# yixuan/LBFGSpp

Measured on AMD Instinct MI355X. Metric: L-BFGS iterations/sec at n=10^8, m=10; achieved HBM GB/s vs peak, higher is better.
Workload: dtype f64; 1 GPU; north-star: extended Rosenbrock n=100000000 m=10 f64 LineSearchMoreThuente, x0 from counter hash; n=100000000, m=10, history_full=True, fevals_total=111, apply_Hv_persistent_launches=82

## Files before the change

include/LBFGSB.h:

```cpp
#ifndef LBFGSX_DROPIN_LBFGSB_H
#define LBFGSX_DROPIN_LBFGSB_H

#include <algorithm>
#include <cmath>
#include <limits>
#include <stdexcept>
#include <vector>

#include "LBFGSpp/BFGSMat.h"
#include "LBFGSpp/Cauchy.h"
#include "LBFGSpp/Device.h"
#include "LBFGSpp/Interop.h"
#include "LBFGSpp/LineSearchMoreThuente.h"
#include "LBFGSpp/Param.h"
#include "LBFGSpp/SubspaceMin.h"

namespace LBFGSpp {

template <typename Scalar, template <class> class LineSearch = LineSearchMoreThuente>
class LBFGSBSolver
{
    const LBFGSBParam<Scalar>& m_param;
    DeviceState<Scalar> m_dev;
    BFGSMatB<Scalar> m_bfgs;
// ... 69 lines not shown
        m_stats.gcp_total_s += gcp.t_total;
        detail::check(lbfgsx_b_dir_from_xcp(c, 1));
        constexpr Scalar eps = std::numeric_limits<Scalar>::epsilon();

        int k = 1;
        for (;;)
        {
            detail::Range range_iteration("lbfgsb:iteration");
            detail::check(lbfgsx_ls_begin(c));
            double dgd = 0, smax = 0;
            if (ev.builtin_id() >= 0 && !ev.reduce)
                detail::check(lbfgsx_b_dg_maxstep_trial(c, ev.builtin_id(), double(std::min(Scalar(1), m_param.max_step)), &dgd, &smax));
            else
                detail::check(lbfgsx_b_dg_maxstep(c, &dgd, &smax));
            Scalar dg = Scalar(dgd), step_max = Scalar(smax);
            if (dg >= Scalar(0) || step_max <= m_param.min_step)
            {
                detail::check(lbfgsx_b_dir_from_xcp(c, 0));
                m_bfgs.reset(c, m_param.m);
                detail::check(lbfgsx_b_dg_maxstep(c, &dgd, &smax));
                dg = Scalar(dgd);
                step_max = Scalar(smax);
                m_stats.resets++;
            }
            step_max = std::min(m_param.max_step, step_max);
            Scalar step = Scalar(1);
            step = std::min(step, step_max);
            const auto t_ls = std::chrono::steady_clock::now();
            ev.trial_written = false;
            try
            {
                detail::Range range_ls("lbfgsb:line_search");
                detail::run_line_search<Scalar, LineSearch<Scalar>, HostVec>(ev, m_param, step_max, step, fx, dg);
            }
            catch (...)
            {
                m_nfev = ev.nfev();
                if (ev.trial_written)
                    m_x_at_throw = LBFGSX_VEC_XT;
                throw;
            }
            m_nfev = ev.nfev();
            m_stats.linesearch_s += std::chrono::duration<double>(std::chrono::steady_clock::now() - t_ls).count();

            double pg = 0, x2 = 0, syd = 0, yyd = 0;
            detail::check(lbfgsx_b_post_linesearch_build(c, Cauchy<Scalar>::build_tau(gcp), &pg, &x2, &syd, &yyd));
            m_projgnorm = Scalar(pg);
            if (m_projgnorm <= m_param.epsilon || m_projgnorm <= m_param.epsilon_rel * sqrt(Scalar(x2)))
                return k;
            if (fpast > 0)
            {
                const Scalar old = m_fx[size_t(k % fpast)];
                if (k >= fpast && abs(old - fx) <= m_param.delta * std::max(std::max(abs(fx), abs(old)), Scalar(1)))
                    return k;
                m_fx[size_t(k % fpast)] = fx;
            }
            if (m_param.max_iterations != 0 && k >= m_param.max_iterations)
                return k;

            const auto t_corr = std::chrono::steady_clock::now();
            if (Scalar(syd) > eps * Scalar(yyd))
                m_bfgs.add_correction_begin(Scalar(syd), Scalar(yyd), m_defer_dots);
            m_stats.correction_s += std::chrono::duration<double>(std::chrono::steady_clock::now() - t_corr).count();

            detail::check(lbfgsx_b_force_bounds_deferred(c));
            {
                detail::Range range_gcp("lbfgsb:cauchy_point");
                Cauchy<Scalar>::get_cauchy_point(m_bfgs, gcp);
            }
            m_stats.gcp_crossings += gcp.crossings;
            m_stats.gcp_dev_crossings += gcp.dev_crossings;
            m_stats.gcp_sort_fallbacks = gcp.sort_fallbacks;
            m_stats.gcp_partial_sorts += (gcp.sorted < gcp.nord_total) ? 1 : 0;
            m_stats.gcp_searches++;
            m_stats.gcp_nord += gcp.nord_total;
            m_stats.gcp_sorted += gcp.sorted;
            m_stats.gcp_build_s += gcp.t_build;
            m_stats.gcp_fetch_s += gcp.t_fetch;
            m_stats.gcp_total_s += gcp.t_total;
            typename SubspaceMin<Scalar>::Stats st;
            const auto t_sub = std::chrono::steady_clock::now();
            {
                detail::Range range_sub("lbfgsb:subspace_min");
                SubspaceMin<Scalar>::subspace_minimize(m_bfgs, gcp, m_param.max_submin, &st);
            }
            m_stats.submin_s += std::chrono::duration<double>(std::chrono::steady_clock::now() - t_sub).count();
            m_stats.submin_calls++;
            m_stats.submin_sweeps += st.sweeps;
            m_stats.submin_unconverged += st.converged ? 0 : 1;
            m_stats.submin_fused_sweeps += st.fused_sweeps;
            m_stats.gram_carried = m_bfgs.carried_grams() - m_carried0;
            m_stats.rhs_identities = m_bfgs.rhs_identities() - m_ident0;
            if (m_trace_phases)
                std::fprintf(stderr, "[lbfgsb] it %d: ls %.3f ms (cum) corr %.3f gcp %.3f (build %.3f fetch %.3f) submin %.3f | crossings %lld dev %lld sweeps %lld\n",
                             k, m_stats.linesearch_s * 1e3, m_stats.correction_s * 1e3, m_stats.gcp_total_s * 1e3,
                             m_stats.gcp_build_s * 1e3, m_stats.gcp_fetch_s * 1e3, m_stats.submin_s * 1e3,
                             m_stats.gcp_crossings, m_stats.gcp_dev_crossings, m_stats.submin_sweeps);
            if (m_iter_hook)
                m_iter_hook(k);
            k++;
        }
    }
    const bool m_defer_dots = [] {
        const char* e = std::getenv("LBFGSX_CORR_DEFER");
        return !(e && e[0] == '0');
    }();
    const bool m_trace_phases = std::getenv("LBFGSX_TRACE_PHASES") != nullptr;

public:
    LBFGSBSolver(const LBFGSBParam<Scalar>& param) : m_param(param) { m_param.check_param(); }

    void set_device(int device) { m_device = device; }
    void set_trace(std::function<void(int, Scalar, DeviceState<Scalar>&)> cb) { m_trace = std::move(cb); }
    void set_iteration_hook(std::function<void(int)> cb) { m_iter_hook = std::move(cb); }
    DeviceState<Scalar>& device_state() { return m_dev; }
    int num_evaluations() const { return m_nfev; }
    const Stats& stats() const { return m_stats; }

    template <typename Foo, typename Vec>
    inline int minimize(Foo& f, Vec& x, Scalar& fx, const Vec& lb, const Vec& ub)
    {
        const std::int64_t n = std::int64_t(x.size());
        if (std::int64_t(lb.size()) != n || std::int64_t(ub.size()) != n)
            throw std::invalid_argument("'lb' and 'ub' must have the same size as 'x'");
        m_dev.ensure(n, m_param.m, LBFGSX_FLAG_BOUNDED, m_device);
        m_dev.upload(LBFGSX_VEC_X, x.data());
        m_dev.upload(LBFGSX_VEC_LB, lb.data());
        m_dev.upload(LBFGSX_VEC_UB, ub.data());
        int k = 0;
        m_x_at_throw = LBFGSX_VEC_X;
        try
        {
            k = run<Foo, Vec>(f, fx);
        }
        catch (...)
        {
            (void) lbfgsx_download(m_dev.ctx(), m_x_at_throw, x.data());
            throw;
        }
        m_dev.download(LBFGSX_VEC_X, x.data());
        return k;
    }

    template <typename Foo>
    inline int minimize_resident(Foo& f, std::int64_t n, Scalar& fx)
    {
        m_dev.ensure(n, m_param.m, LBFGSX_FLAG_BOUNDED, m_device);
        return run<Foo, std::vector<Scalar> >(f, fx);
    }
    void prepare_resident(std::int64_t n)
    {
        m_dev.ensure(n, m_param.m, LBFGSX_FLAG_BOUNDED, m_device);
        detail::check(lbfgsx_b_reserve(m_dev.ctx()));
    }

    const detail::ResultVector<Scalar>& final_grad() const
    {
        m_grad_host.resize(m_dev.size());
        m_dev.download(LBFGSX_VEC_G, m_grad_host.data());
        return m_grad_host;
    }
    Scalar final_grad_norm() const { return m_projgnorm; }
};

}

#endif
```

include/LBFGSpp/SubspaceMin.h:

```cpp
#ifndef LBFGSX_DROPIN_SUBSPACE_MIN_H
#define LBFGSX_DROPIN_SUBSPACE_MIN_H

#include <cstdint>
#include <cstdlib>
#include <limits>
#include <vector>

#include "BFGSMat.h"
#include "Cauchy.h"

namespace LBFGSpp {

template <typename Scalar>
class SubspaceMin
{
    static bool linear_coef(const BFGSMatB<Scalar>& bfgs, const typename Cauchy<Scalar>::Result& gcp, std::vector<double>& coef)
    {
        const int nc = bfgs.num_corrections();
        if (nc < 1 || gcp.nact < 1 || gcp.nfree < 1)
            return false;
        std::vector<Scalar> rhs;
        if (gcp.nact <= gcp.nfree)
            bfgs.Wtv(LBFGSX_VS_DRT, LBFGSX_ST_NEWACT, false, rhs);
        else
        {
            bfgs.Wtv(LBFGSX_VS_DRT, LBFGSX_ST_FREE, false, rhs);
            for (int j = 0; j < 2 * nc; j++)
                rhs[size_t(j)] = gcp.vecc[size_t(j)] - rhs[size_t(j)];
        }
        bfgs.Mv_scaled(rhs, coef);
        return true;
    }

    static bool PtBQv_coef(const BFGSMatB<Scalar>& bfgs, int qmask, int vsel, std::int64_t nP, std::int64_t nQ,
                           std::vector<double>& coef)
    {
        if (bfgs.num_corrections() < 1 || nP < 1 || nQ < 1)
            return false;
        std::vector<Scalar> WQtv;
        std::int64_t nnz = 0;
        bfgs.Wtv(vsel, qmask, false, WQtv, &nnz);
        if (nnz < 1)
            return false;
        bfgs.Mv_scaled(WQtv, coef);
        return true;
    }

public:
    struct Stats
    {
        int sweeps = 0;
        bool converged = true;
        int fused_sweeps = 0;
    };

    static void subspace_minimize(const BFGSMatB<Scalar>& bfgs, const typename Cauchy<Scalar>::Result& gcp, int maxit,
                                  Stats* stats = nullptr)
    {
        lbfgsx_ctx* c = bfgs.ctx();
        const Scalar theta = bfgs.theta();
        detail::check(lbfgsx_b_sub_begin(c));
        const std::int64_t nfree = gcp.nfree;
        if (nfree < 1)
            return;

        std::vector<double> lcoef;
        const bool has_lin = linear_coef(bfgs, gcp, lcoef);
        bfgs.gram_cache_reset();
        const char* fuse_env = std::getenv("LBFGSX_SUB_FUSE");
        const bool fuse = !(fuse_env && fuse_env[0] == '0');
        const char* os_env = std::getenv("LBFGSX_LU_ONE_SIDED");
        const bool one_sided = !(os_env && os_env[0] == '0');
        std::int64_t s7[7] = {0, 0, 0, 0, 0, 0, 0};
        bool swept = false;
        if (fuse)
            detail::check(lbfgsx_b_set_compaction(c, 1));
        bfgs.solve_PtBP(LBFGSX_ST_FREE, nfree, LBFGSX_VS_NEG_CF, LBFGSX_GP_LINEAR,
                        has_lin ? lcoef.data() : nullptr, nullptr, nullptr, 0,
                        true, 0, -1, fuse ? s7 : nullptr, true, &swept);
        std::int64_t cnt[4];
        std::int64_t nL = 0, nU = 0, nP = 0;
        auto take = [&](const std::int64_t* a, const std::int64_t* b2) {
            nL = a[0] + (b2 ? b2[0] : 0);
            nU = a[1] + (b2 ? b2[1] : 0);
            nP = a[2] + (b2 ? b2[2] : 0);
            for (int q = 0; q < 4; q++)
                cnt[q] = a[3 + q] + (b2 ? b2[3 + q] : 0);
        };
        int nfused = swept ? 1 : 0;
        if (swept)
            take(s7, nullptr);
        else if (fuse)
            detail::check(lbfgsx_b_sub_sweep_begin(c, 1, &nL, &nU, &nP, cnt));
        else
            detail::check(lbfgsx_b_sub_check(c, cnt));
        if (cnt[0] == 0)
        {
            detail::check(lbfgsx_b_sub_op(c, LBFGSX_SO_ASSIGN_Y));
            return;
        }
        if (!fuse)
            detail::check(lbfgsx_b_sub_op(c, LBFGSX_SO_SAVE_FALLBACK));

        int k;
        for (k = 0; k < maxit; k++)
        {
            swept = false;
            if (!fuse)
            {
                detail::check(lbfgsx_b_sub_partition(c, &nL, &nU, &nP));
                if (nP > 0)
                    detail::check(lbfgsx_b_sub_op(c, LBFGSX_SO_RHS_INIT));
            }
            const bool need_mult = (nL > 0 || nU > 0);
            std::vector<Scalar> Fy;
            bool have_Fy = false;
            if (nP > 0)
            {
                std::vector<double> cl, cu;
                bool hasL, hasU;
                std::vector<Scalar> wl, wu;
                std::int64_t zl = 0, zu = 0;
                if ((one_sided ? (nL > 0 || nU > 0) : (nL > 0 && nU > 0)) && bfgs.Wtv_lu(wl, zl, wu, zu))
                {
                    hasL = zl >= 1;
                    hasU = zu >= 1;
                    if (hasL)
                        bfgs.Mv_scaled(wl, cl);
                    if (hasU)
                        bfgs.Mv_scaled(wu, cu);
                }
                else
                {
                    hasL = PtBQv_coef(bfgs, LBFGSX_ST_L, LBFGSX_VS_LBOUND, nP, nL, cl);
                    hasU = PtBQv_coef(bfgs, LBFGSX_ST_U, LBFGSX_VS_UBOUND, nP, nU, cu);
                }
                bfgs.solve_PtBP(LBFGSX_ST_P, nP, LBFGSX_VS_NEG_RHS, (hasL || hasU) ? LBFGSX_GP_RHS : LBFGSX_GP_NONE,
                                hasL ? cl.data() : nullptr, hasU ? cu.data() : nullptr, need_mult ? &Fy : nullptr,
                                LBFGSX_ST_FREE, false, LBFGSX_ST_L | LBFGSX_ST_U, nL + nU,
                                (fuse && need_mult && k + 1 < maxit) ? s7 : nullptr, false, &swept);
                have_Fy = need_mult;
            }
            if (need_mult)
            {
                if (!have_Fy)
                    bfgs.Wtv(LBFGSX_VS_Y, LBFGSX_ST_FREE, false, Fy);
                std::vector<double> coef;
                bfgs.Mv_scaled(Fy, coef);
                const double* cf = (bfgs.num_corrections() < 1) ? nullptr : coef.data();
                if (swept)
                {
                    std::int64_t t7[7];
                    detail::check(lbfgsx_b_lu_sweep(c, cf, double(theta), t7));
                    take(s7, t7);
                    nfused++;
// ... 50 lines not shown
```

include/lbfgsx.h:

```cpp
#ifndef LBFGSX_H
#define LBFGSX_H

#include <stddef.h>
#include <stdint.h>

#ifdef __cplusplus
extern "C" {
#endif

typedef struct lbfgsx_ctx lbfgsx_ctx;

enum { LBFGSX_F64 = 0, LBFGSX_F32 = 1 };
enum { LBFGSX_OBJ_NONE = -1, LBFGSX_OBJ_DIAG_QUAD = 0, LBFGSX_OBJ_EXT_ROSENBROCK = 1,
       LBFGSX_OBJ_BOUND = 64  };
enum
{
    LBFGSX_OK = 0,
    LBFGSX_E_INVALID = -1,
    LBFGSX_E_LOGIC = -2,
    LBFGSX_E_RUNTIME = -3,
    LBFGSX_E_HIP = -4,
    LBFGSX_E_NOGPU = -5,
    LBFGSX_E_USER = -6
};
// ... 42 lines not shown
int lbfgsx_bfgs_download_history(lbfgsx_ctx* c, void* S_out, void* Y_out, int* ncorr, int* ptr, double* theta);
int lbfgsx_apply_Hv(lbfgsx_ctx* c, int v_which, double a, double* dg);

int lbfgsx_eval(lbfgsx_ctx* c, int objective, double* fx, double* gnorm2, double* xnorm2);
int lbfgsx_norms(lbfgsx_ctx* c, double* gnorm2, double* xnorm2);
int lbfgsx_ls_begin(lbfgsx_ctx* c);
int lbfgsx_trial(lbfgsx_ctx* c, int objective, double step, double* fx, double* dg);
int lbfgsx_trial_point(lbfgsx_ctx* c, double step);
int lbfgsx_trial_dg(lbfgsx_ctx* c, double* dg);
int lbfgsx_ls_keep_trial_as_lo(lbfgsx_ctx* c);
int lbfgsx_ls_end(lbfgsx_ctx* c, int use_lo);
int lbfgsx_post_linesearch(lbfgsx_ctx* c, double* gnorm2, double* xnorm2, double* sy, double* yy);
int lbfgsx_commit_correction(lbfgsx_ctx* c);
int lbfgsx_post_linesearch_spec(lbfgsx_ctx* c, double a, double* gnorm2, double* xnorm2, double* sy, double* yy);
int lbfgsx_spec_counts(const lbfgsx_ctx* c, int64_t out[3]);
typedef struct lbfgsx_objective lbfgsx_objective;
int lbfgsx_objective_compile(lbfgsx_objective** out, int dtype, int K, const char* body, char* log, size_t log_len);
void lbfgsx_objective_destroy(lbfgsx_objective* obj);
long long lbfgsx_objective_source(int dtype, int K, const char* body, char* out, size_t len);
int lbfgsx_objective_info(const lbfgsx_objective* obj, long long out[8]);
int lbfgsx_objective_K(const lbfgsx_objective* obj);
int lbfgsx_objective_dtype(const lbfgsx_objective* obj);
int lbfgsx_objective_bind(lbfgsx_ctx* c, const lbfgsx_objective* obj, const void* const p[4], const double cs[8], int* id);
int lbfgsx_objective_upload(lbfgsx_ctx* c, int slot, const void* host, void** dev);
int lbfgsx_objective_bound(const lbfgsx_ctx* c, const void* p[4]);
enum { LBFGSX_FORM_TERM = 0, LBFGSX_FORM_CHAIN = 1, LBFGSX_FORM_GRID = 2 };
int lbfgsx_objective_compile_chain(lbfgsx_objective** out, int dtype, int K, const char* body, char* log, size_t log_len);
long long lbfgsx_objective_source_chain(int dtype, int K, const char* body, char* out, size_t len);
int lbfgsx_objective_form(const lbfgsx_objective* obj);
int lbfgsx_objective_compile_grid(lbfgsx_objective** out, int dtype, const char* body, char* log, size_t log_len);
long long lbfgsx_objective_source_grid(int dtype, const char* body, char* out, size_t len);
int lbfgsx_objective_bind_grid(lbfgsx_ctx* c, const lbfgsx_objective* obj, int64_t rows, int64_t cols, const void* const p[4],
                               const double cs[8], int* id);
int lbfgsx_objective_shape(const lbfgsx_ctx* c, int64_t* rows, int64_t* cols);
int lbfgsx_device(const lbfgsx_ctx* c);
int lbfgsx_device_push(const lbfgsx_ctx* c, int* prev);
int lbfgsx_device_pop(int prev);
int lbfgsx_persist_counts(const lbfgsx_ctx* c, int64_t out[4]);
int lbfgsx_debug_persist_fault(lbfgsx_ctx* c);
int lbfgsx_counters(int64_t out[3], int reset);
int lbfgsx_counters_ex(int64_t out[8], int reset);
int lbfgsx_poll_counts(const lbfgsx_ctx* c, int64_t out[2]);
int lbfgsx_poll_counts_ex(const lbfgsx_ctx* c, int64_t out[4]);
void lbfgsx_range_push(const char* name);
void lbfgsx_range_pop(void);

int lbfgsx_gs_post_linesearch(lbfgsx_ctx* c, double scal[7], double* sdots, double* gdots, double* ydots);
int lbfgsx_gs_set_history_dtype(lbfgsx_ctx* c, int dtype);
int lbfgsx_gs_direction(lbfgsx_ctx* c, const double* coef, double coef_g, double* dg);

enum
{
    LBFGSX_ST_FREE = 1, LBFGSX_ST_NEWACT = 2, LBFGSX_ST_L = 4, LBFGSX_ST_U = 8, LBFGSX_ST_P = 16
};
enum
{
    LBFGSX_VS_DRT = 0,
    LBFGSX_VS_NEG_CF = 1,
    LBFGSX_VS_NEG_RHS = 2,
    LBFGSX_VS_LBOUND = 3,
    LBFGSX_VS_UBOUND = 4,
    LBFGSX_VS_Y = 5
};
enum
{
    LBFGSX_CB_LINEAR = 0,
    LBFGSX_CB_SOLVE = 1,
    LBFGSX_CB_RHS_ADD = 2,
    LBFGSX_CB_LAMBDA = 3,
    LBFGSX_CB_MU = 4
};
enum
{
    LBFGSX_SO_SAVE_FALLBACK = 0, LBFGSX_SO_RHS_INIT = 1, LBFGSX_SO_ASSIGN_Y = 2, LBFGSX_SO_CLAMP_Y = 3,
    LBFGSX_SO_CLAMP_FB = 4, LBFGSX_SO_ASSIGN_FB = 5
};
int lbfgsx_b_force_bounds(lbfgsx_ctx* c);
int lbfgsx_b_force_bounds_deferred(lbfgsx_ctx* c);
int lbfgsx_b_eval(lbfgsx_ctx* c, int objective, double* fx, double* projgnorm, double* xnorm2);
int lbfgsx_b_norms(lbfgsx_ctx* c, double* projgnorm, double* xnorm2);
int lbfgsx_b_dg_maxstep(lbfgsx_ctx* c, double* dg, double* step_max);
int lbfgsx_b_dg_maxstep_trial(lbfgsx_ctx* c, int objective, double step0, double* dg, double* step_max);
int lbfgsx_b_trial_ahead_counts(const lbfgsx_ctx* c, int64_t out[2]);
int lbfgsx_b_post_linesearch(lbfgsx_ctx* c, double* projgnorm, double* xnorm2, double* sy, double* yy);
int lbfgsx_b_post_linesearch_build(lbfgsx_ctx* c, double tau, double* projgnorm, double* xnorm2, double* sy, double* yy);
int lbfgsx_b_post_build_counts(int64_t out[2], int reset);
int lbfgsx_b_psel_counts(int64_t out[1], int reset);
int lbfgsx_b_correction_dots(lbfgsx_ctx* c, double* sdots, double* ydots);
int lbfgsx_b_correction_dots_defer(lbfgsx_ctx* c);
int lbfgsx_b_cauchy_build(lbfgsx_ctx* c, int64_t* nfree, int64_t* nord, double* dd, double* wtd);
int lbfgsx_b_cauchy_chunk(lbfgsx_ctx* c, int64_t first, int64_t count, double* brk, double* g, double* z, int* idx,
                          double* wrows);
int lbfgsx_b_cauchy_build_partial(lbfgsx_ctx* c, double tau, int64_t* nfree, int64_t* nord, int64_t* nsorted, double* dd,
                                  double* wtd);
int lbfgsx_b_cauchy_sort_full(lbfgsx_ctx* c);
int lbfgsx_b_cauchy_scan(lbfgsx_ctx* ctx, int64_t first, int64_t count, int64_t nord, const double* Mmat, double theta,
                         double t_prev, const double* state_in, int64_t* exit_at, double* state_out);
int lbfgsx_b_cauchy_finish(lbfgsx_ctx* c, double t_cross, double tfinal, int crossed_all, int64_t* nact, int64_t* nfree);
int lbfgsx_b_sub_begin(lbfgsx_ctx* c);
int lbfgsx_b_wtv(lbfgsx_ctx* c, int vsel, int mask, double* out, int64_t* nnz);
int lbfgsx_b_gram(lbfgsx_ctx* c, int mask, double* gram);
int lbfgsx_b_gram_fused(lbfgsx_ctx* c, int mask, int vsel, double* gram, double* wtv);
enum { LBFGSX_GP_NONE = 0, LBFGSX_GP_RHS = 1, LBFGSX_GP_LINEAR = 2 };
int lbfgsx_b_gram_fused_ex(lbfgsx_ctx* c, int mask, int vsel_id, int prologue, const double* coef1, const double* coef2,
                           double* gram, double* wtv);
int lbfgsx_b_gram_fused_dd(lbfgsx_ctx* c, int mask, int vsel_id, int prologue, const double* coef1, const double* coef2,
                           double* gram, double* wtv, double* gram_dd);
int lbfgsx_b_wtv_prologue(lbfgsx_ctx* c, int mask, int vsel_id, int prologue, const double* coef1, const double* coef2,
                          double* wtv);
int lbfgsx_b_solve_wty(lbfgsx_ctx* c, int pmask, int vsel, const double* coef, double theta, int fmask, double* wty);
int lbfgsx_b_wcombine(lbfgsx_ctx* c, int mode, int mask, int vsel, const double* coef, double theta);
int lbfgsx_b_sub_partition(lbfgsx_ctx* c, int64_t* nL, int64_t* nU, int64_t* nP);
int lbfgsx_b_sub_check(lbfgsx_ctx* c, int64_t counts[4]);
int lbfgsx_b_sub_sweep_begin(lbfgsx_ctx* c, int first, int64_t* nL, int64_t* nU, int64_t* nP, int64_t counts[4]);
int lbfgsx_b_wtv_lu(lbfgsx_ctx* c, double* out_l, int64_t* nnz_l, double* out_u, int64_t* nnz_u);
int lbfgsx_b_wtv_lu_c(lbfgsx_ctx* c, double* out_l, int64_t* nnz_l, double* out_u, int64_t* nnz_u, double* negc_dd);
int lbfgsx_b_free_delta(lbfgsx_ctx* c, int64_t* n_enter, int64_t* n_leave);
int lbfgsx_b_gram_list_dd(lbfgsx_ctx* c, int which, double* gram_dd);
int lbfgsx_b_gram_pairs_dd(lbfgsx_ctx* c, int mask, int vsel, int prologue, const double* coef1, const double* coef2,
                           int npairs, const int* pair_i, const int* pair_j, int refresh_slot, double* out_dd);
int lbfgsx_b_gram_pairs_max(lbfgsx_ctx* c);
int lbfgsx_b_gram_last_vrow_dd(lbfgsx_ctx* c, double* out_dd);
int lbfgsx_b_set_compaction(lbfgsx_ctx* c, int enable);
int lbfgsx_b_compact_vec_counts(int64_t out[4], int reset);
int lbfgsx_b_reserve(lbfgsx_ctx* c);
int lbfgsx_b_solve_sweep(lbfgsx_ctx* c, int first, int vsel, const double* coef, double theta, double* wty, int64_t sums[7]);
int lbfgsx_b_solve_sweep_rhs(lbfgsx_ctx* c, int first, int vsel, const double* coef, double theta, const double* rhs_c1,
                             const double* rhs_c2, double* wty, int64_t sums[7]);
int lbfgsx_b_solve_sweep_rhs_ready(lbfgsx_ctx* c);
int lbfgsx_b_lu_sweep(lbfgsx_ctx* c, const double* coef, double theta, int64_t sums[7]);
int lbfgsx_b_sub_op(lbfgsx_ctx* c, int op);
int lbfgsx_b_download_state(lbfgsx_ctx* c, unsigned char* host);
int lbfgsx_b_dot_drt_g(lbfgsx_ctx* c, double* dg);
int lbfgsx_b_dir_from_xcp(lbfgsx_ctx* c, int normalize);

typedef struct lbfgsx_batch lbfgsx_batch;
typedef struct
{
    int active;
    int mode;
    int x_in;
    int x_out;
    int col_u;
    int col_w;
    int i_num, i_den, i_num2, i_theta, i_out;
    float pad;
    double step;
} lbfgsx_bat_desc;
enum
{
    LBFGSX_BAT_EVAL = 0, LBFGSX_BAT_TRIAL = 1, LBFGSX_BAT_POST = 2, LBFGSX_BAT_TWOLOOP = 3,
    LBFGSX_BAT_POINT = 4, LBFGSX_BAT_GDOT = 5, LBFGSX_BAT_NORMS = 6
};
typedef struct
{
    int active;
    int x_in;
    int ncorr;
    int pcol[32];
} lbfgsx_bat_hvdesc;
enum
{
    LBFGSX_BAT_IT_POST = 1,
    LBFGSX_BAT_IT_POST_ONLY = 2,
    LBFGSX_BAT_IT_TRIAL = 4,
    LBFGSX_BAT_IT_TRIAL_ONLY = 8
// ... 73 lines not shown
```

lbfgspp_amd/_lib.py:

```python
import ctypes as C
import os

HERE = os.path.dirname(os.path.abspath(__file__))

F64, F32 = 0, 1
OBJ_DIAG_QUAD, OBJ_EXT_ROSENBROCK = 0, 1
OBJ_BOUND = 64
LS_NOCEDAL_WRIGHT, LS_MORE_THUENTE, LS_BACKTRACKING, LS_BRACKETING = 0, 1, 2, 3
ALGO_LBFGS, ALGO_LBFGSB = 0, 1
RECURSION_VECTOR, RECURSION_GRAM_SPACE, RECURSION_GRAM_SPACE_F32H = 0, 1, 2
FLAG_BOUNDED = 1
(VEC_X, VEC_G, VEC_XP, VEC_GP, VEC_D, VEC_XT, VEC_GT, VEC_A, VEC_B, VEC_LB, VEC_UB, VEC_XCP) = range(12)
E_INVALID, E_LOGIC, E_RUNTIME, E_HIP, E_NOGPU, E_USER = -1, -2, -3, -4, -5, -6


class Params(C.Structure):
    _fields_ = [("m", C.c_int), ("epsilon", C.c_double), ("epsilon_rel", C.c_double), ("past", C.c_int),
                ("delta", C.c_double), ("max_iterations", C.c_int), ("linesearch", C.c_int),
                ("max_linesearch", C.c_int), ("min_step", C.c_double), ("max_step", C.c_double),
                ("ftol", C.c_double), ("wolfe", C.c_double), ("max_submin", C.c_int)]


class Result(C.Structure):
    _fields_ = [("niter", C.c_int), ("nfev", C.c_int), ("fx", C.c_double), ("gnorm", C.c_double),
# ... 46 lines not shown
        f = getattr(lib, name)
        f.restype = res
        f.argtypes = list(args)
        return f

    sig(core, "lbfgsx_last_error", C.c_char_p)
    sig(core, "lbfgsx_version", C.c_char_p)
    sig(core, "lbfgsx_device_count", i32)
    sig(core, "lbfgsx_create", i32, C.POINTER(vp), i32, i64, i32, i32, i32)
    sig(core, "lbfgsx_destroy", None, vp)
    sig(core, "lbfgsx_set_stream", i32, vp, vp)
    sig(core, "lbfgsx_sync", i32, vp)
    sig(core, "lbfgsx_n", i64, vp)
    sig(core, "lbfgsx_vec", vp, vp, i32)
    sig(core, "lbfgsx_upload", i32, vp, i32, vp)
    sig(core, "lbfgsx_download", i32, vp, i32, vp)
    sig(core, "lbfgsx_gather", i32, vp, i32, i64, pd)
    sig(core, "lbfgsx_gen_diag_quad", i32, vp, dbl, C.c_uint64)
    sig(core, "lbfgsx_gen_rosen_x0", i32, vp, C.c_uint64)
    sig(core, "lbfgsx_fill", i32, vp, i32, dbl)
    sig(core, "lbfgsx_bfgs_reset", i32, vp)
    sig(core, "lbfgsx_bfgs_ncorr", i32, vp)
    sig(core, "lbfgsx_bfgs_theta", dbl, vp)
    sig(core, "lbfgsx_bfgs_add_correction_host", i32, vp, vp, vp)
    sig(core, "lbfgsx_bfgs_download_history", i32, vp, vp, vp, C.POINTER(i32), C.POINTER(i32), pd)
    sig(core, "lbfgsx_apply_Hv", i32, vp, i32, dbl, pd)
    sig(core, "lbfgsx_eval", i32, vp, i32, pd, pd, pd)
    sig(core, "lbfgsx_norms", i32, vp, pd, pd)
    sig(core, "lbfgsx_ls_begin", i32, vp)
    sig(core, "lbfgsx_trial", i32, vp, i32, dbl, pd, pd)
    sig(core, "lbfgsx_trial_point", i32, vp, dbl)
    sig(core, "lbfgsx_trial_dg", i32, vp, pd)
    sig(core, "lbfgsx_ls_keep_trial_as_lo", i32, vp)
    sig(core, "lbfgsx_ls_end", i32, vp, i32)
    sig(core, "lbfgsx_post_linesearch", i32, vp, pd, pd, pd, pd)
    sig(core, "lbfgsx_commit_correction", i32, vp)
    sig(core, "lbfgsx_gs_post_linesearch", i32, vp, pd, pd, pd, pd)
    sig(core, "lbfgsx_gs_set_history_dtype", i32, vp, i32)
    sig(core, "lbfgsx_gs_direction", i32, vp, pd, dbl, pd)
    sig(core, "lbfgsx_timing_enable", i32, vp, i32)
    sig(core, "lbfgsx_timing_read", i32, vp, pd, C.POINTER(i64), pd, C.POINTER(i64))
    sig(core, "lbfgsx_stream_probe", i32, vp, i32, pd, pd)
    sig(core, "lbfgsx_selftest_reduce", i32, vp, i32, i32, i32, pd)
    sig(core, "lbfgsx_post_linesearch_spec", i32, vp, dbl, pd, pd, pd, pd)
    sig(core, "lbfgsx_rccl_allgather_records", i32, C.POINTER(i32), i32, vp, i64, i64, C.POINTER(vp))
    sig(core, "lbfgsx_device_download", i32, i32, vp, i64, vp)
    sig(core, "lbfgsx_device_free", None, i32, vp)
    sig(core, "lbfgsx_spec_counts", i32, vp, C.POINTER(i64 * 3))
    sig(core, "lbfgsx_counters", i32, C.POINTER(i64 * 3), i32)
    sig(core, "lbfgsx_counters_ex", i32, C.POINTER(i64 * 8), i32)
    sig(core, "lbfgsx_poll_counts", i32, vp, C.POINTER(i64 * 2))
    sig(core, "lbfgsx_poll_counts_ex", i32, vp, C.POINTER(i64 * 4))
    sig(core, "lbfgsx_b_compact_vec_counts", i32, C.POINTER(i64 * 4), i32)
    sig(core, "lbfgsx_b_reserve", i32, vp)
    sig(core, "lbfgsx_device", i32, vp)
    sig(core, "lbfgsx_persist_counts", i32, vp, C.POINTER(i64 * 4))
    sig(core, "lbfgsx_debug_persist_fault", i32, vp)

    sig(sol, "lbfgsx_solver_create", i32, C.POINTER(vp), i32, i32, i32, C.POINTER(Params), i32)
    sig(sol, "lbfgsx_solver_create_error", C.c_char_p)
    sig(sol, "lbfgsx_solver_destroy", None, vp)
    sig(sol, "lbfgsx_solver_prepare", i32, vp, i64)
    sig(sol, "lbfgsx_solver_ctx", vp, vp)
    sig(sol, "lbfgsx_solver_set_recursion", i32, vp, i32)
    sig(sol, "lbfgsx_solver_set_allreduce", i32, vp, ALLREDUCE, vp)
    sig(sol, "lbfgsx_solver_set_devices", i32, vp, C.POINTER(i32), i32)
    sig(core, "lbfgsx_comm_unique_id", i32, C.c_char_p)
    sig(core, "lbfgsx_comm_create_rank", i32, C.POINTER(vp), i32, i32, i32, C.c_char_p)
    sig(core, "lbfgsx_comm_create_local", i32, C.POINTER(vp), C.POINTER(i32), i32)
    sig(core, "lbfgsx_comm_allreduce_sum", i32, vp, i32, pd, i32)
    sig(core, "lbfgsx_comm_abort", i32, vp)
    sig(core, "lbfgsx_comm_abort_from", i32, vp, i32)
    sig(core, "lbfgsx_comm_first_abort", i32, vp)
    sig(core, "lbfgsx_b_gram_pairs_max", i32, vp)
    sig(core, "lbfgsx_b_post_linesearch_build", i32, vp, dbl, pd, pd, pd, pd)
    sig(core, "lbfgsx_b_post_build_counts", i32, C.POINTER(i64 * 2), i32)
    sig(core, "lbfgsx_b_psel_counts", i32, C.POINTER(i64 * 1), i32)
    sig(core, "lbfgsx_b_dg_maxstep_trial", i32, vp, i32, dbl, pd, pd)
    sig(core, "lbfgsx_b_solve_sweep_rhs", i32, vp, i32, i32, pd, dbl, pd, pd, pd, C.POINTER(i64 * 7))
    sig(core, "lbfgsx_b_solve_sweep_rhs_ready", i32, vp)
    sig(core, "lbfgsx_b_gram_last_vrow_dd", i32, vp, pd)
    sig(core, "lbfgsx_b_wtv_lu_c", i32, vp, pd, C.POINTER(i64), pd, C.POINTER(i64), pd)
    sig(core, "lbfgsx_b_trial_ahead_counts", i32, vp, C.POINTER(i64 * 2))
    sig(core, "lbfgsx_comm_info", i32, vp, C.POINTER(i32 * 4))
    sig(core, "lbfgsx_comm_calls", i64, vp, i32)
    sig(core, "lbfgsx_comm_hook_arg", vp, vp, i32)
    sig(core, "lbfgsx_comm_destroy", None, vp)
    sig(core, "lbfgsx_set_shard", i32, vp, i64, i64)
    sig(sol, "lbfgsx_solver_set_iteration_hook", i32, vp, ITER_HOOK, vp)
    sig(sol, "lbfgsx_batch_minimize", i32, i32, i32, i32, C.POINTER(Params), i32, i64, i64, i64, C.c_uint64, i32, i32,
        C.POINTER(BatchItem))
    sig(sol, "lbfgsx_batch_minimize_lockstep", i32, i32, C.POINTER(Params), i64, i64, i32, C.c_uint64, i32,
        C.POINTER(BatchItem), vp, C.c_char_p, i32)
    sig(sol, "lbfgsx_batch_minimize_lockstep_multi", i32, i32, C.POINTER(Params), i64, i64, i32, C.c_uint64,
        C.POINTER(i32), i32, C.POINTER(BatchItem), vp, C.c_char_p, i32)
    sig(sol, "lbfgsx_batch_minimize_lockstep_ex", i32, i32, i32, i32, dbl, C.POINTER(Params), i64, i64, i32, C.c_uint64,
        C.POINTER(i32), i32, C.POINTER(BatchItem), vp, C.c_char_p, i32)
    sig(sol, "lbfgsx_lockstep_create", i32, C.POINTER(vp), i32, i32, C.POINTER(Params), i64, i32, i32, i32, C.c_char_p, i32)
    sig(sol, "lbfgsx_lockstep_minimize", i32, vp, i32, dbl, C.c_uint64, i64, C.POINTER(BatchItem), vp, C.POINTER(dbl * 8),
        C.c_char_p, i32)
    sig(sol, "lbfgsx_lockstep_destroy", None, vp)
    sig(sol, "lbfgsx_lockstep_set_timing", i32, vp, i32)
    sig(sol, "lbfgsx_solver_hessians", i32, vp, vp, vp)
    sig(sol, "lbfgsx_solver_stats", i32, vp, C.POINTER(C.c_longlong * 8))
    sig(sol, "lbfgsx_solver_stats2", i32, vp, C.POINTER(C.c_longlong * 8))
    sig(sol, "lbfgsx_solver_stats3", i32, vp, C.POINTER(C.c_longlong * 8))
    sig(sol, "lbfgsx_solver_minimize", i32, vp, i32, i64, vp, vp, vp, vp, vp, C.POINTER(Trace), C.POINTER(Result))
    sig(sol, "lbfgsx_solver_minimize_fn", i32, vp, i64, OBJECTIVE_FN, vp, vp, vp, vp, C.POINTER(Trace), C.POINTER(Result))
    sig(sol, "lbfgsx_lockstep_minimize_fn", i32, vp, vp, BATCH_OBJECTIVE_FN, vp, C.POINTER(BatchItem), vp, C.POINTER(dbl * 8),
        C.c_char_p, i32)
    sig(core, "lbfgsx_objective_compile", i32, C.POINTER(vp), i32, i32, C.c_char_p, C.c_char_p, C.c_size_t)
    sig(core, "lbfgsx_objective_destroy", None, vp)
    sig(core, "lbfgsx_objective_source", C.c_longlong, i32, i32, C.c_char_p, C.c_char_p, C.c_size_t)
    sig(core, "lbfgsx_objective_info", i32, vp, C.POINTER(C.c_longlong * 8))
    sig(core, "lbfgsx_objective_compile_chain", i32, C.POINTER(vp), i32, i32, C.c_char_p, C.c_char_p, C.c_size_t)
    sig(core, "lbfgsx_objective_source_chain", C.c_longlong, i32, i32, C.c_char_p, C.c_char_p, C.c_size_t)
    sig(core, "lbfgsx_objective_form", i32, vp)
    sig(core, "lbfgsx_objective_K", i32, vp)
    sig(core, "lbfgsx_objective_dtype", i32, vp)
    sig(core, "lbfgsx_objective_bind", i32, vp, vp, C.POINTER(vp * 4), C.POINTER(dbl * 8), C.POINTER(i32))
    sig(core, "lbfgsx_objective_upload", i32, vp, i32, vp, C.POINTER(vp))
    sig(core, "lbfgsx_objective_bound", i32, vp, C.POINTER(vp * 4))
    sig(sol, "lbfgsx_solver_minimize_obj", i32, vp, vp, i64, C.POINTER(vp * 4), i32, C.POINTER(dbl * 8), vp, vp, vp,
        C.POINTER(Trace), C.POINTER(Result))
    sig(core, "lbfgsx_objective_compile_grid", i32, C.POINTER(vp), i32, C.c_char_p, C.c_char_p, C.c_size_t)
    sig(core, "lbfgsx_objective_source_grid", C.c_longlong, i32, C.c_char_p, C.c_char_p, C.c_size_t)
    sig(core, "lbfgsx_objective_bind_grid", i32, vp, vp, i64, i64, C.POINTER(vp * 4), C.POINTER(dbl * 8), C.POINTER(i32))
    sig(core, "lbfgsx_objective_shape", i32, vp, C.POINTER(i64), C.POINTER(i64))
    sig(sol, "lbfgsx_solver_minimize_grid", i32, vp, vp, i64, i64, C.POINTER(vp * 4), i32, C.POINTER(dbl * 8), vp, vp, vp,
        C.POINTER(Trace), C.POINTER(Result))
    _core, _solver = core, sol
    return core, sol


def last_error():
    core, _ = load()
    return core.lbfgsx_last_error().decode()


_EXC = {E_INVALID: ValueError, E_LOGIC: ArithmeticError, E_RUNTIME: RuntimeError, E_HIP: RuntimeError,
        E_NOGPU: RuntimeError, E_USER: RuntimeError}


def check(rc, msg=None):
    if rc != 0:
        raise _EXC.get(rc, RuntimeError)(msg if msg is not None else last_error())


def require_torch(who):
    try:
        import torch
    except ImportError as e:
        raise ImportError("%s needs PyTorch (ROCm build): its callable receives torch tensors that alias the library's "
                          "device vectors" % who) from e
    return torch


class _DeviceMemory:

    def __init__(self, ptr, shape, np_dtype, strides):
        import numpy as np
        self.__cuda_array_interface__ = {"shape": tuple(shape), "typestr": np.dtype(np_dtype).str, "data": (int(ptr), False),
                                         "version": 2, "strides": strides}


def device_tensor(ptr, shape, np_dtype, device, row_stride=None):
# ... 6 lines not shown
```

lbfgspp_amd/csrc/lbfgsb.hip:

```cpp
#include <algorithm>
#include <atomic>
#include <cmath>
#include <cstdlib>
#include <cstdio>
#include <cstring>

#define LBFGSB_TU "lbfgsb"
#include "lbfgsb_state.hpp"

namespace lbfgsx {

static std::atomic<int64_t> g_cv_starts{0}, g_cv_backs{0}, g_wtdc_runs{0}, g_stash_hits{0};
void count_cv_start() { g_cv_starts.fetch_add(1, std::memory_order_relaxed); }
void count_wtdc_run() { g_wtdc_runs.fetch_add(1, std::memory_order_relaxed); }
void count_stash_hit() { g_stash_hits.fetch_add(1, std::memory_order_relaxed); }

int cv_alloc(lbfgsx_ctx* c)
{
    lbfgsb_state* b = c->bstate;
    if (b->cv_buf && b->cv_cap >= c->ld)
        return LBFGSX_OK;
    if (b->cv_buf)
        (void) hipFree(b->cv_buf);
    b->cv_buf = nullptr;
// ... 92 lines not shown
int fetch_T(lbfgsx_ctx* c, int idx, int k, double* out)
{
    if (idx == c->sl.out(0) && c->outmap_dev)
    {
        LBFGSX_HIP(lbfgsx::poll_wait(c));
        const volatile T* h = static_cast<const volatile T*>(c->outmap_host);
        for (int i = 0; i < k; i++)
            out[i] = double(h[i]);
        return LBFGSX_OK;
    }
    LBFGSX_HIP(lbfgsx::copy_async(c->hout, P<T>(c->sc) + idx, sizeof(T) * size_t(k), hipMemcpyDeviceToHost, c->stream));
    LBFGSX_HIP(lbfgsx::stream_sync(c->stream));
    const T* h = static_cast<const T*>(c->hout);
    for (int i = 0; i < k; i++)
        out[i] = double(h[i]);
    return LBFGSX_OK;
}

template int fetch_T<float>(lbfgsx_ctx*, int, int, double*);
template int fetch_T<double>(lbfgsx_ctx*, int, int, double*);

int bounded_alloc(lbfgsx_ctx* c)
{
    lbfgsb_state* b = new lbfgsb_state();
    c->bstate = b;
    const size_t vbytes = size_t(c->ld) * c->esz;
    void** vecs[] = {&b->brk, &b->dvec, &b->cF, &b->y, &b->yfb, &b->lam, &b->mu, &b->rhs, &b->keys_in, &b->keys_out};
    for (void** v : vecs)
        LBFGSX_HIP(hipMalloc(v, vbytes));
    LBFGSX_HIP(hipMalloc(reinterpret_cast<void**>(&b->st), size_t(c->ld)));
    LBFGSX_HIP(hipMemset(b->st, 0, size_t(c->ld)));
    LBFGSX_HIP(hipMalloc(reinterpret_cast<void**>(&b->vals_in), sizeof(int) * size_t(c->ld)));
    LBFGSX_HIP(hipMalloc(reinterpret_cast<void**>(&b->vals_out), sizeof(int) * size_t(c->ld)));
    LBFGSX_HIP(hipMalloc(reinterpret_cast<void**>(&b->phys_dev), sizeof(int) * size_t(c->m + 1)));
    if (c->outmap_dev)
    {
        LBFGSX_HIP(hipHostMalloc(reinterpret_cast<void**>(&b->dout_host), sizeof(double) * lbfgsb_state::kDout, hipHostMallocMapped | hipHostMallocCoherent));
        std::memset(b->dout_host, 0, sizeof(double) * lbfgsb_state::kDout);
        LBFGSX_HIP(hipHostGetDevicePointer(reinterpret_cast<void**>(&b->dout), b->dout_host, 0));
    }
    else
        LBFGSX_HIP(hipMalloc(reinterpret_cast<void**>(&b->dout), sizeof(double) * lbfgsb_state::kDout));
    LBFGSX_HIP(hipMalloc(&b->coef_dev, sizeof(double) * 80));
    b->lu_cap = unsigned(std::min<int64_t>(c->n, int64_t(1) << 20));
    LBFGSX_HIP(hipMalloc(reinterpret_cast<void**>(&b->lu_list), sizeof(int) * 2 * size_t(b->lu_cap)));
    LBFGSX_HIP(hipMalloc(reinterpret_cast<void**>(&b->lu_cnt), sizeof(unsigned)));
    LBFGSX_HIP(hipMemset(b->lu_cnt, 0, sizeof(unsigned)));
    if (const char* e = getenv("LBFGSX_SWEEP_SOLVE_FUSE"))
        b->sweep_fuse = atoi(e) != 0;
    if (const char* e = getenv("LBFGSX_COMPACT_FREE"))
        b->wf_use = atoi(e) != 0;
    if (const char* e = getenv("LBFGSX_SPLIT"))
        b->split = atoi(e) != 0;
    if (const char* e = getenv("LBFGSX_FINISH_FUSE"))
        b->fin_fuse = atoi(e) != 0;
    if (const char* e = getenv("LBFGSX_NEWACT_CAP"))
        b->na_cap = unsigned(std::max(1, std::min(1 << 20, atoi(e))));
    LBFGSX_HIP(hipMalloc(reinterpret_cast<void**>(&b->na_list), sizeof(int) * size_t(b->na_cap)));
    LBFGSX_HIP(hipMalloc(reinterpret_cast<void**>(&b->na_cnt), sizeof(unsigned)));
    LBFGSX_HIP(hipMemset(b->na_cnt, 0, sizeof(unsigned)));
    LBFGSX_HIP(hipMalloc(reinterpret_cast<void**>(&b->xp1), sizeof(double) * size_t(kMaxGridX) * kMaxSumsX * 2));
    LBFGSX_HIP(hipMalloc(reinterpret_cast<void**>(&b->xp2), sizeof(double) * size_t(kMaxGridX / kGroupX) * kMaxSumsX * 2));
    LBFGSX_HIP(hipMalloc(reinterpret_cast<void**>(&b->xtickets), sizeof(unsigned) * (2 + kMaxGridX / kGroupX)));
    LBFGSX_HIP(hipMemset(b->xtickets, 0, sizeof(unsigned) * (2 + kMaxGridX / kGroupX)));
    b->gtile = std::max(3, xl::gram_kpb(2 * c->m + 1));
    if (const char* e = getenv("LBFGSX_COMPACT_VEC"))
        b->cv_use = atoi(e) != 0;
    if (const char* e = getenv("LBFGSX_WTD_COMPACT"))
        b->wtdc_use = atoi(e) != 0;
    if (const char* e = getenv("LBFGSX_SELECT_INLINE"))
        b->psel_use = atoi(e) != 0;
    if (const char* e = getenv("LBFGSX_POST_BUILD"))
        b->pb_use = atoi(e) != 0;
    if (const char* e = getenv("LBFGSX_TRIAL_AHEAD"))
        b->st_use = atoi(e) != 0;
    if (const char* e = getenv("LBFGSX_RHS_IDENTITY"))
        b->rhs_identity = atoi(e) != 0;
    if (const char* e = getenv("LBFGSX_CHUNK_AHEAD"))
        b->gpre_use = atoi(e) != 0;
    if (const char* e = getenv("LBFGSX_DELTA_AHEAD"))
        b->fd_use = atoi(e) != 0;
    if (const char* e = getenv("LBFGSX_LIST12"))
        b->list12 = atoi(e) != 0;
    if (const char* e = getenv("LBFGSX_PSEL_SMALL"))
        b->psel_small = atoi(e) != 0;
    if (const char* e = getenv("LBFGSX_SELECT_CAP"))
        b->psel_cap = unsigned(std::max(1, std::min(1 << 24, atoi(e))));
    if (const char* e = getenv("LBFGSX_SYNC_MERGE"))
        b->stash_use = atoi(e) != 0;
    if (const char* e = getenv("LBFGSX_WTD_LIST_CAP"))
        b->wtdc_cap = unsigned(std::max(1, std::min(1 << 20, atoi(e))));
    LBFGSX_HIP(hipMalloc(reinterpret_cast<void**>(&b->colmax), sizeof(unsigned long long) * 2 * size_t(c->m + 1)));
    LBFGSX_HIP(hipMemset(b->colmax, 0, sizeof(unsigned long long) * 2 * size_t(c->m + 1)));
    b->colmax_ok.assign(size_t(c->m + 1), 0);
    const size_t bytes = sort_pairs_tmp_bytes(c);
    if (const char* e = getenv("LBFGSX_GRAM"))
    {
        b->gram_i8 = (std::strcmp(e, "i8") == 0);
        if (const char* e2 = getenv("LBFGSX_GRAM_I8_MIN"))
            b->i8_min_tot = std::max(1, atoi(e2));
        b->gram_mode = (std::strcmp(e, "blocked") == 0) ? 2 : 0;
        if (!b->gram_i8 && b->gram_mode == 0 && e[0] != 0 && std::strcmp(e, "dd") != 0)
        {
            static bool warned = false;
            if (!warned)
                fprintf(stderr, "lbfgsx: LBFGSX_GRAM=%s is not a Gram kernel (i8, blocked, dd): using the default\n", e);
            warned = true;
        }
    }
    if (const char* e = getenv("LBFGSX_GCP_CHAIN"))
        b->chain_host = std::strcmp(e, "scan") != 0;
    if (const char* e = getenv("LBFGSX_MULTIDOT"))
        b->multidot_chunked = (std::strcmp(e, "chunked") == 0);
    {
        hipDeviceProp_t prop;
        if (hipGetDeviceProperties(&prop, c->device) == hipSuccess && prop.multiProcessorCount > 0)
            b->num_cus = prop.multiProcessorCount;
    }
    const size_t gent = size_t(b->gtile) * 256;
    LBFGSX_HIP(hipMalloc(reinterpret_cast<void**>(&b->gram_partial), sizeof(double) * size_t(lbfgsb_state::kGramBlocks) * gent * 2));
    LBFGSX_HIP(hipMalloc(reinterpret_cast<void**>(&b->gram_partial2), sizeof(double) * 32 * gent * 2));
    if (c->outmap_dev)
    {
        LBFGSX_HIP(hipHostMalloc(reinterpret_cast<void**>(&b->gram_dd_host), sizeof(double) * gent * 2, hipHostMallocMapped | hipHostMallocCoherent));
        LBFGSX_HIP(hipHostGetDevicePointer(reinterpret_cast<void**>(&b->gram_dd), b->gram_dd_host, 0));
        LBFGSX_HIP(hipHostMalloc(reinterpret_cast<void**>(&b->stash_host), sizeof(double) * 3 * (gent * 3), hipHostMallocMapped | hipHostMallocCoherent));
        LBFGSX_HIP(hipHostGetDevicePointer(reinterpret_cast<void**>(&b->stash_dev), b->stash_host, 0));
        LBFGSX_HIP(hipHostMalloc(reinterpret_cast<void**>(&b->gram_out_host), sizeof(double) * gent, hipHostMallocMapped | hipHostMallocCoherent));
        LBFGSX_HIP(hipHostGetDevicePointer(reinterpret_cast<void**>(&b->gram_out), b->gram_out_host, 0));
    }
    else
    {
        LBFGSX_HIP(hipMalloc(reinterpret_cast<void**>(&b->gram_out), sizeof(double) * gent));
        LBFGSX_HIP(hipMalloc(reinterpret_cast<void**>(&b->gram_dd), sizeof(double) * gent * 2));
    }
    b->sort_tmp_bytes = bytes;
    LBFGSX_HIP(hipMalloc(&b->sort_tmp, bytes ? bytes : 16));
    return LBFGSX_OK;
}

void bounded_free(lbfgsx_ctx* c)
{
    lbfgsb_state* b = c->bstate;
    if (!b)
        return;
    void* ptrs[] = {b->brk, b->dvec, b->cF, b->y, b->yfb, b->lam, b->mu, b->rhs, b->keys_in, b->keys_out, b->st,
                    b->vals_in, b->vals_out, b->phys_dev, b->dout, b->coef_dev, b->sort_tmp, b->g_brk,
                    b->g_g, b->g_z, b->g_w, b->g_idx, b->gram_partial, b->gram_partial2, b->gram_out, b->gram_dd,
                    b->s_brk, b->s_g, b->s_z, b->s_W, b->s_P, b->s_C, b->s_chain, b->s_ts, b->s_off,
                    b->s_small, b->s_exit, b->pk, b->pv, b->pcount, b->sel_tmp};
    if (b->h_chain)
        (void) hipHostFree(b->h_chain);
    if (b->exit_map_host)
        (void) hipHostFree(b->exit_map_host);
    if (b->gout_host)
        (void) hipHostFree(b->gout_host);
    if (b->g_host)
        (void) hipHostFree(b->g_host);
    if (b->fd_host)
        (void) hipHostFree(b->fd_host);
    (void) hipFree(b->lu_list);
    (void) hipFree(b->wf_pos);
    (void) hipFree(b->wtdc_list);
    (void) hipFree(b->wtdc_cnt);
    (void) hipFree(b->psel_list);
    (void) hipFree(b->psel_cnt);
    (void) hipFree(b->psel_tmp);
    for (hipEvent_t ev : b->chain_ev)
        if (ev)
            (void) hipEventDestroy(ev);
    (void) hipFree(b->fprev);
    (void) hipFree(b->dl_enter);
    (void) hipFree(b->dl_leave);
    (void) hipFree(b->dl_cnt);
    (void) hipFree(b->wf);
    (void) hipFree(b->wf_idx);
    (void) hipFree(b->wf_cnt);
    (void) hipFree(b->wf_base);
    (void) hipFree(b->wf_tmp);
    (void) hipFree(b->lu_cnt);
    (void) hipFree(b->colmax);
    (void) hipFree(b->i8_part);
    (void) hipFree(b->i8_partv);
    (void) hipFree(b->i8_vsum);
    for (void* p : ptrs)
    {
        if ((p == b->dout && b->dout_host) || (p == b->gram_out && b->gram_out_host) || (p == b->gram_dd && b->gram_dd_host))
            continue;
        (void) hipFree(p);
    }
    if (b->dout_host)
        (void) hipHostFree(b->dout_host);
    if (b->gram_out_host)
        (void) hipHostFree(b->gram_out_host);
    if (b->gram_dd_host)
        (void) hipHostFree(b->gram_dd_host);
    if (b->stash_host)
        (void) hipHostFree(b->stash_host);
    (void) hipFree(b->cv_buf);
    (void) hipFree(b->na_list);
    (void) hipFree(b->na_cnt);
    (void) hipFree(b->xp1);
    (void) hipFree(b->xp2);
    (void) hipFree(b->xtickets);
    delete b;
    c->bstate = nullptr;
}

RedWsX wsx(lbfgsx_ctx* c)
{
    RedWsX w;
    w.p1 = c->bstate->xp1;
    w.p2 = c->bstate->xp2;
    w.tickets = c->bstate->xtickets;
    w.done = c->ws.done;
    w.seq = c->ws.seq;
    return w;
}
int ensure_keys(lbfgsx_ctx* c)
{
    lbfgsb_state* b = c->bstate;
    if (b->keys_valid && b->vals_iota)
        return LBFGSX_OK;
    const int grid = c->grid_for(c->n);
    DISPATCH_T(c, {
        lbfgsx::model_add(double(c->n) * (2 * sizeof(T) + (b->vals_iota ? 0 : 4)));
        LBFGSX_LAUNCH((k_keys_from_brk<T>), dim3(grid), dim3(kBlock), 0, c->stream, static_cast<const T*>(b->brk),
                      static_cast<T*>(b->keys_in), b->vals_iota ? static_cast<int*>(nullptr) : b->vals_in, c->n);
    });
    LBFGSX_HIP(hipGetLastError());
    b->keys_valid = true;
    b->vals_iota = true;
    return LBFGSX_OK;
}

void wf_rebuilt(lbfgsx_ctx* c)
{
    lbfgsb_state* b = c->bstate;
    b->wf_valid = true;
    b->wf_n = b->nfree_last;
    b->wf_live = true;
    b->wf_ncorr = c->ncorr;
    b->wf_epoch = b->sub_epoch;
}

bool wtdc_ready(lbfgsx_ctx* c, bool assume_defer)
{
    lbfgsb_state* b = c->bstate;
    const int total = 2 * c->ncorr;
    return b->wtdc_use && (b->corr_defer || assume_defer) && (b->split ? (total >= 2 && total <= kColsX) : (total > 8 && total <= 20)) &&
           !b->multidot_chunked && b->wf_use && b->wf_live &&
           (b->wf_ncorr == c->ncorr || b->wf_ncorr + 1 == c->ncorr) && b->wf_epoch == b->sub_epoch && c->n < (int64_t(1) << 31) &&
           b->wf_n >= 4096 && b->wf_n * 4 <= c->n * 3;
}
bool wtdc_prepare(lbfgsx_ctx* c)
{
    lbfgsb_state* b = c->bstate;
    b->wtdc_n = -1;
    if (!wtdc_ready(c))
        return false;
    return wtdc_alloc(c);
}
bool wtdc_alloc(lbfgsx_ctx* c)
{
    lbfgsb_state* b = c->bstate;
    if (!b->wtdc_list)
    {
        if (hipMalloc(reinterpret_cast<void**>(&b->wtdc_list), sizeof(int) * size_t(b->wtdc_cap)) != hipSuccess ||
            hipMalloc(reinterpret_cast<void**>(&b->wtdc_cnt), sizeof(unsigned)) != hipSuccess ||
            hipMemsetAsync(b->wtdc_cnt, 0, sizeof(unsigned), c->stream) != hipSuccess)
        {
            (void) hipGetLastError();
            (void) hipFree(b->wtdc_list);
            (void) hipFree(b->wtdc_cnt);
            b->wtdc_list = nullptr;
            b->wtdc_cnt = nullptr;
            b->wtdc_use = false;
            return false;
        }
    }
    return true;
}

int run_force_bounds(lbfgsx_ctx* c)
{
    c->bstate->pb_valid = false;
    lbfgsx::DeviceGuard dev_guard_(c->device);
    const int grid = c->grid_for(c->n);
    DISPATCH_T(c, {
        LBFGSX_LAUNCH((k_force_bounds<T>), dim3(grid), dim3(kBlock), 0, c->stream, P<T>(c->xb[c->cur]), P<T>(c->lb),
                           P<T>(c->ub), c->n);
    });
    LBFGSX_HIP(hipGetLastError());
    return LBFGSX_OK;
}

int psort_alloc(lbfgsx_ctx* c)
{
    lbfgsb_state* b = c->bstate;
    if (!b->pk)
    {
        const size_t n = size_t(c->n);
        LBFGSX_HIP(hipMalloc(&b->pk, c->esz * n));
        LBFGSX_HIP(hipMalloc(reinterpret_cast<void**>(&b->pv), sizeof(int) * n));
        LBFGSX_HIP(hipMalloc(reinterpret_cast<void**>(&b->pcount), sizeof(unsigned)));
    }
    return LBFGSX_OK;
}

int delta_alloc(lbfgsx_ctx* c)
{
    lbfgsb_state* b = c->bstate;
    if (!b->fprev)
    {
        b->dl_cap = unsigned(std::min<int64_t>(c->n, std::max<int64_t>(int64_t(1) << 14, std::min<int64_t>(int64_t(1) << 20, c->n / 64))));
        LBFGSX_HIP(hipMalloc(reinterpret_cast<void**>(&b->fprev), size_t(c->ld)));
        LBFGSX_HIP(hipMemsetAsync(b->fprev, 0, size_t(c->ld), c->stream));
        LBFGSX_HIP(hipMalloc(reinterpret_cast<void**>(&b->dl_enter), sizeof(int) * size_t(b->dl_cap)));
        LBFGSX_HIP(hipMalloc(reinterpret_cast<void**>(&b->dl_leave), sizeof(int) * size_t(b->dl_cap)));
        LBFGSX_HIP(hipMalloc(reinterpret_cast<void**>(&b->dl_cnt), sizeof(unsigned) * 4));
    }
    return LBFGSX_OK;
}

}

using namespace lbfgsx;

extern "C" {

int lbfgsx_b_reserve(lbfgsx_ctx* c)
{
    lbfgsx::DeviceGuard dev_guard_(c->device);
    int rc = need_bounded(c);
    if (rc)
        return rc;
    lbfgsb_state* b = c->bstate;
    const int m2 = 2 * c->m;
    const int ncap = m2 <= 32 ? std::max(4, (m2 + 3) / 4 * 4) : m2 <= 40 ? 40 : m2 <= 48 ? 48 : m2 <= 64 ? 64 : 80;
    if (m2 <= 80)
    {
        rc = scan_alloc(c, std::min<int64_t>(int64_t(1) << 20, c->n), ncap);
        if (rc)
            return rc;
    }
    rc = psort_alloc(c);
    if (rc)
        return rc;
    rc = delta_alloc(c);
    if (rc)
        return rc;
    if (b->wf_use && c->n >= 4096 && c->n < (int64_t(1) << 31))
        (void) wf_alloc(c);
    if (b->cv_use && b->wf_use)
        (void) cv_alloc(c);
    if (b->wtdc_use)
        (void) wtdc_alloc(c);
    return LBFGSX_OK;
}

int lbfgsx_b_compact_vec_counts(int64_t out[4], int reset)
{
    if (out)
    {
        out[0] = g_cv_starts.load(std::memory_order_relaxed);
        out[1] = g_cv_backs.load(std::memory_order_relaxed);
        out[2] = g_wtdc_runs.load(std::memory_order_relaxed);
        out[3] = g_stash_hits.load(std::memory_order_relaxed);
    }
    if (reset)
    {
        g_cv_starts = 0;
        g_cv_backs = 0;
        g_wtdc_runs = 0;
        g_stash_hits = 0;
    }
    return LBFGSX_OK;
}

int lbfgsx_b_set_compaction(lbfgsx_ctx* c, int enable)
{
    int rc = need_bounded(c);
    if (rc)
        return rc;
    c->bstate->wf_on = enable != 0;
    if (!enable)
        c->bstate->wf_valid = false;
    return LBFGSX_OK;
}

int lbfgsx_b_download_state(lbfgsx_ctx* c, unsigned char* host)
{
    lbfgsx::DeviceGuard dev_guard_(c->device);
    int rc = need_bounded(c);
    if (rc)
        return rc;
    LBFGSX_HIP(lbfgsx::copy_async(host, c->bstate->st, size_t(c->n), hipMemcpyDeviceToHost, c->stream));
    LBFGSX_HIP(lbfgsx::stream_sync(c->stream));
    return LBFGSX_OK;
}

}
```

lbfgspp_amd/csrc/lbfgsb_cauchy.hip:

```cpp
#include <algorithm>
#include <atomic>
#include <cmath>
#include <cstdlib>
#include <cstdio>
#include <cstring>

#include <rocprim/rocprim.hpp>

#include "gcp_scan.cuh"

#define LBFGSB_TU "lbfgsb_cauchy"
#include "lbfgsb_state.hpp"

namespace lbfgsx {

template <class T>
struct KeyLE
{
    T tau;
    __device__ bool operator()(const T& k) const { return k <= tau; }
};
template <class T>
__global__ void k_gather_keys(const T* __restrict__ keys, const int* __restrict__ idx, T* __restrict__ out, int64_t count)
{
// ... 202 lines not shown
        b->psel_list = nullptr;
        b->psel_cnt = nullptr;
        b->psel_tmp = nullptr;
        b->psel_use = false;
        return false;
    }
    b->psel_tmp_bytes = bytes;
    return true;
}
template <class T>
static int partial_sort_tail_t(lbfgsx_ctx* c, unsigned cnt, int64_t* nsorted)
{
    lbfgsb_state* b = c->bstate;
    *nsorted = int64_t(cnt);
    if (cnt == 0)
        return LBFGSX_OK;
    const int grid = int(std::min<int64_t>((int64_t(cnt) + 255) / 256, 1024));
    LBFGSX_LAUNCH((k_gather_keys<T>), dim3(grid), dim3(256), 0, c->stream, b->keys_valid ? P<T>(b->keys_in) : static_cast<T*>(b->brk),
                  b->pv, P<T>(b->pk), int64_t(cnt));
    size_t sbytes = b->sort_tmp_bytes;
    lbfgsx::model_add(double(cnt) * (96.0 + 64.0 + 2 * sizeof(T)));
    LBFGSX_HIP(rocprim::radix_sort_pairs(b->sort_tmp, sbytes, P<T>(b->pk), P<T>(b->keys_out), b->pv, b->vals_out, size_t(cnt), 0,
                                         int(sizeof(T) * 8), c->stream));
    return LBFGSX_OK;
}
template <class T>
static int partial_sort_listed_t(lbfgsx_ctx* c, unsigned cnt, int64_t* nsorted)
{
    lbfgsb_state* b = c->bstate;
    if (b->psel_small && cnt >= 1 && cnt <= unsigned(kPselSmallCap))
    {
        *nsorted = int64_t(cnt);
        g_psel_small++;
        lbfgsx::model_add(double(cnt) * (64.0 + 4 + 2 * (sizeof(T) + 4)));
        LBFGSX_LAUNCH((k_psel_sort_small<T>), dim3(1), dim3(kPselSmallThreads), 0, c->stream, b->psel_list, int(cnt),
                      b->keys_valid ? P<T>(b->keys_in) : static_cast<T*>(b->brk), P<T>(b->keys_out), b->vals_out);
        LBFGSX_HIP(hipGetLastError());
        return LBFGSX_OK;
    }
    if (cnt > 1)
    {
        size_t bytes = b->psel_tmp_bytes;
        int end_bit = 1;
        while (end_bit < 32 && (int64_t(1) << end_bit) < c->n)
            end_bit++;
        LBFGSX_HIP(rocprim::radix_sort_keys(b->psel_tmp, bytes, b->psel_list, b->pv, size_t(cnt), 0, end_bit, c->stream));
    }
    else if (cnt == 1)
        LBFGSX_HIP(lbfgsx::copy_async(b->pv, b->psel_list, sizeof(int), hipMemcpyDeviceToDevice, c->stream));
    return partial_sort_tail_t<T>(c, cnt, nsorted);
}
template <class T>
static int partial_sort_t(lbfgsx_ctx* c, double tau, int64_t* nsorted)
{
    lbfgsb_state* b = c->bstate;
    int rc = partial_select_t<T>(c, tau, nullptr);
    if (rc)
        return rc;
    unsigned cnt = 0;
    LBFGSX_HIP(lbfgsx::copy_async(&cnt, b->pcount, sizeof(unsigned), hipMemcpyDeviceToHost, c->stream));
    LBFGSX_HIP(lbfgsx::stream_sync(c->stream));
    return partial_sort_tail_t<T>(c, cnt, nsorted);
}
static int cauchy_chunk_launch(lbfgsx_ctx* c, int64_t first, int64_t count, bool with_w, int* idx, double** land,
                               std::vector<double>* pageable)
{
    lbfgsb_state* b = c->bstate;
    const int nc = c->ncorr;
    const size_t per = size_t(3 + 2 * nc);
    const size_t per_cap = size_t(3 + 2 * c->m);
    if (count > b->g_cap || c->m != b->g_ncorr)
    {
        void* old[] = {b->g_brk, b->g_idx};
        for (void* p : old)
            (void) hipFree(p);
        b->g_brk = nullptr;
        b->g_idx = nullptr;
        const int64_t cap = std::max<int64_t>(count, b->g_cap);
        LBFGSX_HIP(hipMalloc(reinterpret_cast<void**>(&b->g_brk), sizeof(double) * size_t(cap) * per_cap));
        LBFGSX_HIP(hipMalloc(reinterpret_cast<void**>(&b->g_idx), sizeof(int) * size_t(cap)));
        b->g_cap = cap;
        b->g_ncorr = c->m;
    }
    double* d_brk = b->g_brk;
    double* d_g = d_brk + count;
    double* d_z = d_g + count;
    double* d_w = d_z + count;
    int rc = upload_phys(c);
    if (rc)
        return rc;
    const int grid = int(std::min<int64_t>((count + 255) / 256, 2048));
    DISPATCH_T(c, {
        BVecs<T> bv = bvecs<T>(c);
        LBFGSX_LAUNCH((k_cauchy_gather<T>), dim3(grid), dim3(256), 0, c->stream, bv, P<T>(b->keys_out), b->vals_out, first,
                           count, P<T>(c->S), P<T>(c->Y), c->ld, b->phys_dev, nc, d_brk, d_g, d_z, b->g_idx, d_w);
    });
    LBFGSX_HIP(hipGetLastError());
    const size_t ndbl = size_t(count) * ((nc > 0 && with_w) ? per : size_t(3));
    if (ndbl > b->g_host_cap)
    {
        if (b->g_host)
            (void) hipHostFree(b->g_host);
        b->g_host = nullptr;
        b->g_host_cap = 0;
        const size_t want = std::max<size_t>(ndbl, size_t(1) << 16);
        if (want <= (size_t(1) << 25))
        {
            LBFGSX_HIP(hipHostMalloc(reinterpret_cast<void**>(&b->g_host), sizeof(double) * want, hipHostMallocDefault));
            b->g_host_cap = want;
        }
    }
    *land = b->g_host;
    if (ndbl > b->g_host_cap)
    {
        if (!pageable)
            return LBFGSX_E_INVALID;
        pageable->resize(ndbl);
        *land = pageable->data();
    }
    LBFGSX_HIP(lbfgsx::copy_async(*land, d_brk, sizeof(double) * ndbl, hipMemcpyDeviceToHost, c->stream));
    if (idx)
        LBFGSX_HIP(lbfgsx::copy_async(idx, b->g_idx, sizeof(int) * size_t(count), hipMemcpyDeviceToHost, c->stream));
    return LBFGSX_OK;
}
template <int NC>
static int gcp_scan_nc(lbfgsx_ctx* c, const GcpBufs& gb, int64_t first, int64_t count, int64_t nord, double theta,
                       double t_prev)
{
    lbfgsb_state* b = c->bstate;
    const int nc = c->ncorr;
    const int ntiles = int((count + kGcpTile - 1) / kGcpTile);
    double* M = b->s_small;
    double* initA = M + NC * NC;
    double* initB = initA + NC;
    double* initC = initB + NC + 1;
    double* fin = initC + 1;
    double* out = fin + NC + 1;
    hipStream_t st = c->stream;
    LBFGSX_LAUNCH((k_gcp_a1<NC>), dim3(ntiles), dim3(kGcpTile), 0, st, gb, count, nc, theta, b->s_ts);
    LBFGSX_LAUNCH(k_gcp_tiles, dim3(NC), dim3(64), 0, st, b->s_ts, b->s_off, ntiles, NC, initA, fin);
    LBFGSX_LAUNCH((k_gcp_a3b1<NC>), dim3(ntiles), dim3(kGcpTile), 0, st, gb, count, nc, theta, t_prev, M, b->s_off, b->s_ts);
    LBFGSX_LAUNCH(k_gcp_tiles, dim3(NC + 1), dim3(64), 0, st, b->s_ts, b->s_off, ntiles, NC + 1, initB, fin);
    if (b->chain_host)
    {
        LBFGSX_LAUNCH((k_gcp_b3c1<NC, true>), dim3(ntiles), dim3(kGcpTile), 0, st, gb, count, nc, theta, t_prev, M,
                           b->s_off, b->s_ts, first, nord);
        LBFGSX_HIP(hipGetLastError());
        return LBFGSX_OK;
    }
    LBFGSX_LAUNCH((k_gcp_b3c1<NC, false>), dim3(ntiles), dim3(kGcpTile), 0, st, gb, count, nc, theta, t_prev, M, b->s_off, b->s_ts, first, nord);
    LBFGSX_LAUNCH(k_gcp_tiles, dim3(1), dim3(64), 0, st, b->s_ts, b->s_off, ntiles, 1, initC, fin);
    LBFGSX_LAUNCH(k_gcp_c3, dim3(ntiles), dim3(kGcpTile), 0, st, gb, count, first, nord, b->s_off, b->s_exit);
    LBFGSX_LAUNCH((k_gcp_extract<NC>), dim3(1), dim3(64), 0, st, gb, count, nc, theta, b->s_exit, out);
    LBFGSX_HIP(hipGetLastError());
    return LBFGSX_OK;
}
template <int NC>
static void gcp_extract_nc(lbfgsx_ctx* c, const GcpBufs& gb, int64_t count, double theta)
{
    lbfgsb_state* b = c->bstate;
    LBFGSX_LAUNCH((k_gcp_extract<NC>), dim3(1), dim3(64), 0, c->stream, gb, count, c->ncorr, theta, b->exit_map_dev, b->gout_dev);
}

template <class CT>
static int64_t gcp_chain_host(const double* dt, const double* A, const double* B, int64_t k0, int64_t k1, double& fp, double& fpp)
{
    CT f1 = CT(fp), f2 = CT(fpp);
    for (int64_t k = k0; k < k1; k++)
    {
        f1 = f1 + CT(dt[k]) * f2;
        f1 = f1 + CT(A[k]);
        f2 = f2 - CT(B[k]);
        const CT dn = CT(dt[k + 1]);
        if (dn > CT(0) && !(-f1 / f2 >= dn))
        {
            fp = double(f1);
            fpp = double(f2);
            return k;
        }
    }
    fp = double(f1);
// ... 115 lines not shown
        return rc;
    lbfgsb_state* b = c->bstate;
    const bool force = b->force_pending;
    b->force_pending = false;
    const int grid = c->grid_for(c->n);
    double r[5] = {0, 0, 0, -1, -1};
    int64_t ns = 0;
    const bool tau_ok = tau > 0.0 && std::isfinite(tau);
    const bool sel_inline = tau_ok && b->psel_use && b->psel_last >= 0 && b->psel_last <= lbfgsb_state::kPselMax &&
                            c->n < (int64_t(1) << 31) && psel_alloc(c);
    const bool sel_ahead = !sel_inline && b->stash_use && b->dout_host && tau_ok;
    DISPATCH_T(c, {
        BVecs<T> bv = bvecs<T>(c);
        const bool wc = wtdc_prepare(c);
        const int newest = (c->ptr + c->m - 1) % c->m;
        const bool from_post = b->pb_valid && b->pb_cur == c->cur && b->pb_tau == tau && b->pb_sel_inline == sel_inline &&
                               b->pb_wc == wc && !sel_ahead && (!force || b->pb_r[5] == 0.0);
        b->pb_valid = false;
        if (from_post)
        {
            for (int i = 0; i < 5; i++)
                r[i] = b->pb_r[i];
            count_pb_hit();
        }
        else
        {
        if (!sel_ahead)
            lbfgsx::poll_arm(c);
        lbfgsx::model_add(double(c->n) * (7 * sizeof(T) + 4));
        b->keys_valid = b->vals_iota = true;
        LBFGSX_LAUNCH((k_cauchy_build<T>), dim3(grid), dim3(kBlock), 0, c->stream, bv, P<T>(b->keys_in), b->vals_in, c->n,
                           c->ws, b->dout, force ? P<T>(c->xb[c->cur]) : static_cast<T*>(nullptr),
                           wc ? static_cast<const T*>(c->col(c->S, c->phys[size_t(newest)])) : static_cast<const T*>(nullptr),
                           wc ? b->wf_pos : static_cast<const int*>(nullptr), b->wtdc_list, b->wtdc_cnt, b->wtdc_cap, T(tau),
                           sel_inline ? b->psel_list : static_cast<int*>(nullptr), b->psel_cnt, b->psel_cap);
        LBFGSX_HIP(hipGetLastError());
        if (sel_ahead)
        {
            rc = partial_select_t<T>(c, tau, reinterpret_cast<unsigned*>(b->dout + 60));
            if (rc)
                return rc;
        }
        rc = fetch_doubles(c, sel_inline ? 5 : wc ? 4 : 3, r);
        if (rc)
            return rc;
        }
        b->wtdc_n = wc ? int64_t(r[3]) : -1;
        ns = int64_t(r[2]);
        if (r[2] > 0)
        {
            if (tau_ok)
            {
                if (sel_inline && r[4] >= 0 && r[4] <= double(b->psel_cap))
                    rc = partial_sort_listed_t<T>(c, unsigned(r[4]), &ns);
                else if (sel_ahead)
                    rc = partial_sort_tail_t<T>(c, *reinterpret_cast<const volatile unsigned*>(b->dout_host + 60), &ns);
                else
                    rc = partial_sort_t<T>(c, tau, &ns);
                if (rc)
                    return rc;
            }
            else
            {
                {
                    const int rk = ensure_keys(c);
                    if (rk)
                        return rk;
                }
                size_t bytes = b->sort_tmp_bytes;
                lbfgsx::model_add(96.0 * double(c->n));
                LBFGSX_HIP(rocprim::radix_sort_pairs(b->sort_tmp, bytes, P<T>(b->keys_in), P<T>(b->keys_out), b->vals_in,
                                                     b->vals_out, size_t(c->n), 0, int(sizeof(T) * 8), c->stream));
            }
        }
        if (wtd && c->ncorr > 0)
        {
            b->gpre_valid = false;
            if (b->gpre_use && ns >= 1)
            {
                double* land = nullptr;
                const int64_t cnt = std::min<int64_t>(512, ns);
                if (cauchy_chunk_launch(c, 0, cnt, true, nullptr, &land, nullptr) == LBFGSX_OK)
                {
                    b->gpre_valid = true;
                    b->gpre_count = cnt;
                    b->gpre_nc = c->ncorr;
                }
                else
                    (void) hipGetLastError();
            }
            rc = cauchy_wtd(c, wtd);
            if (rc)
            {
                b->gpre_valid = false;
                return rc;
            }
        }
    });
    b->psel_last = tau_ok ? ns : int64_t(-1);
    if (dd) *dd = r[0];
    if (nfree) *nfree = int64_t(r[1]);
    if (nord) *nord = int64_t(r[2]);
    if (nsorted) *nsorted = ns;
    return LBFGSX_OK;
}

int lbfgsx_b_cauchy_sort_full(lbfgsx_ctx* c)
{
    lbfgsx::DeviceGuard dev_guard_(c->device);
    int rc = need_bounded(c);
    if (rc)
        return rc;
    lbfgsb_state* b = c->bstate;
    b->gpre_valid = false;
    rc = ensure_keys(c);
    if (rc)
        return rc;
    DISPATCH_T(c, {
        size_t bytes = b->sort_tmp_bytes;
        lbfgsx::model_add(96.0 * double(c->n));
        LBFGSX_HIP(rocprim::radix_sort_pairs(b->sort_tmp, bytes, P<T>(b->keys_in), P<T>(b->keys_out), b->vals_in, b->vals_out,
                                             size_t(c->n), 0, int(sizeof(T) * 8), c->stream));
    });
    return LBFGSX_OK;
}

int lbfgsx_b_cauchy_chunk(lbfgsx_ctx* c, int64_t first, int64_t count, double* brk, double* g, double* z, int* idx,
                          double* wrows)
{
    lbfgsx::DeviceGuard dev_guard_(c->device);
    int rc = need_bounded(c);
    if (rc)
        return rc;
    lbfgsb_state* b = c->bstate;
    if (count <= 0)
        return LBFGSX_OK;
    const int nc = c->ncorr;
    double* land = nullptr;
    std::vector<double> pageable;
    const bool ahead = b->gpre_valid && first == 0 && count == b->gpre_count && nc == b->gpre_nc && !idx && (wrows || nc == 0);
    b->gpre_valid = false;
    if (ahead)
        land = b->g_host;
    else
    {
        rc = cauchy_chunk_launch(c, first, count, wrows != nullptr, idx, &land, &pageable);
        if (rc)
            return rc;
        LBFGSX_HIP(lbfgsx::stream_sync(c->stream));
    }
    std::memcpy(brk, land, sizeof(double) * size_t(count));
    std::memcpy(g, land + count, sizeof(double) * size_t(count));
    std::memcpy(z, land + 2 * count, sizeof(double) * size_t(count));
    if (nc > 0 && wrows)
        std::memcpy(wrows, land + 3 * count, sizeof(double) * size_t(count) * size_t(2 * nc));
    return LBFGSX_OK;
}

int lbfgsx_b_cauchy_scan(lbfgsx_ctx* c, int64_t first, int64_t count, int64_t nord, const double* Mmat, double theta,
                         double t_prev, const double* state_in, int64_t* exit_at, double* state_out)
{
    lbfgsx::DeviceGuard dev_guard_(c->device);
    int rc = need_bounded(c);
    if (rc)
        return rc;
    lbfgsb_state* b = c->bstate;
    const int nc = c->ncorr, nc2 = 2 * nc;
    if (nc2 > 80 || count < 1 || first < 0 || first + count > nord)
    {
        set_error("lbfgsx_b_cauchy_scan: needs 2*ncorr <= 80 and a non-empty range inside the sorted list");
        return LBFGSX_E_INVALID;
    }
    const int NC = nc2 <= 32 ? std::max(4, (nc2 + 3) / 4 * 4) : nc2 <= 40 ? 40 : nc2 <= 48 ? 48 : nc2 <= 64 ? 64 : 80;
    rc = scan_alloc(c, count, NC);
    if (rc)
        return rc;
    rc = upload_phys(c);
    if (rc)
        return rc;
    std::vector<double> hbuf(size_t(80 * 80 + 6 * 88), 0.0);
    double* h = hbuf.data();
    for (int i = 0; i < nc2; i++)
        for (int j = 0; j < nc2; j++)
            h[i * NC + j] = Mmat[size_t(j) * size_t(nc2) + size_t(i)];
    double* initA = h + NC * NC;
    double* initB = initA + NC;
    double* initC = initB + NC + 1;
    for (int j = 0; j < nc2; j++)
    {
        initA[j] = state_in[j];
        initB[j] = state_in[nc2 + j];
    }
    initB[NC] = state_in[2 * nc2 + 1];
    initC[0] = state_in[2 * nc2];
    const size_t nsmall = size_t(NC * NC + NC + NC + 1 + 1);
    LBFGSX_HIP(lbfgsx::copy_async(b->s_small, h, sizeof(double) * nsmall, hipMemcpyHostToDevice, c->stream));
    if (!b->chain_host)
        LBFGSX_HIP(hipMemsetAsync(b->s_exit, 0xFF, sizeof(unsigned long long), c->stream));
    const int grid = int(std::min<int64_t>((count + 256) / 256, 2048));
    DISPATCH_T(c, {
        LBFGSX_LAUNCH((k_gcp_gather<T>), dim3(grid), dim3(256), 0, c->stream, bvecs<T>(c), P<T>(b->keys_out), b->vals_out,
                           first, count, nord, P<T>(c->S), P<T>(c->Y), c->ld, b->phys_dev, nc, b->s_brk, b->s_g, b->s_z, b->s_W,
                           b->s_cap);
    });
    b->s_fp = b->s_chain;
    b->s_dfp = b->s_chain + (count + 1);
    b->s_fpp = b->s_chain + 2 * (count + 1);
    GcpBufs gb = {b->s_brk, b->s_g, b->s_z, b->s_W, b->s_P, b->s_C, b->s_fpp, b->s_dfp, b->s_fp, b->s_cap};
    switch (NC)
    {
    case 4: rc = gcp_scan_nc<4>(c, gb, first, count, nord, theta, t_prev); break;
    case 8: rc = gcp_scan_nc<8>(c, gb, first, count, nord, theta, t_prev); break;
    case 12: rc = gcp_scan_nc<12>(c, gb, first, count, nord, theta, t_prev); break;
    case 16: rc = gcp_scan_nc<16>(c, gb, first, count, nord, theta, t_prev); break;
    case 20: rc = gcp_scan_nc<20>(c, gb, first, count, nord, theta, t_prev); break;
    case 24: rc = gcp_scan_nc<24>(c, gb, first, count, nord, theta, t_prev); break;
    case 28: rc = gcp_scan_nc<28>(c, gb, first, count, nord, theta, t_prev); break;
    case 32: rc = gcp_scan_nc<32>(c, gb, first, count, nord, theta, t_prev); break;
    case 40: rc = gcp_scan_nc<40>(c, gb, first, count, nord, theta, t_prev); break;
    case 48: rc = gcp_scan_nc<48>(c, gb, first, count, nord, theta, t_prev); break;
    case 64: rc = gcp_scan_nc<64>(c, gb, first, count, nord, theta, t_prev); break;
    default: rc = gcp_scan_nc<80>(c, gb, first, count, nord, theta, t_prev); break;
    }
    if (rc)
        return rc;
    double fp_h = state_in[2 * nc2], fpp_h = state_in[2 * nc2 + 1];
// ... 139 lines not shown
```

lbfgspp_amd/csrc/lbfgsb_gram.hip:

```cpp
#include <algorithm>
#include <atomic>
#include <cmath>
#include <cstdlib>
#include <cstdio>
#include <cstring>

#include "gram_i8.cuh"

#define LBFGSB_TU "lbfgsb_gram"
#include "lbfgsb_state.hpp"

namespace lbfgsx {

int bounded_note_column(lbfgsx_ctx* c, int col)
{
    lbfgsb_state* b = c->bstate;
    if (!b || !b->gram_i8 || col < 0 || col > c->m)
        return LBFGSX_OK;
    unsigned long long* cmx = b->colmax + 2 * size_t(col);
    LBFGSX_HIP(hipMemsetAsync(cmx, 0, 2 * sizeof(unsigned long long), c->stream));
    const int grid = c->grid_for(c->n);
    DISPATCH_T(c, {
        LBFGSX_LAUNCH((k_colmax2<T>), dim3(grid), dim3(kBlock), 0, c->stream, P<T>(c->col(c->S, col)), P<T>(c->col(c->Y, col)),
                           c->n, cmx + 1, cmx + 0);
// ... 263 lines not shown
    lbfgsb_state* b = c->bstate;
    int which[32];
    for (int k = 0; k < tot; k++)
        which[k] = k;
    Cols<T, 32> cl = (gr.in_idx || by_pos) ? wf_cols<T>(c, tot) : col_list<T, 32>(c, which, tot);
    const int per_cu = (NA == 1 && NC <= 20) ? 2 : 1;
    const int grid = std::max(1, std::min(std::min(c->grid_for(nrows), b->num_cus * per_cu), c->ws.maxGrid));
    LBFGSX_LAUNCH((k_vrows<T, NC, NA>), dim3(grid), dim3(kBlock), 0, c->stream, cl, tot, by_pos ? *by_pos : bvecs<T>(c), vsel_id,
                  mask, nrows, c->ws, b->gram_out, b->gram_out + 256, pro, gr, col_a, col_b);
    LBFGSX_HIP(hipGetLastError());
    return LBFGSX_OK;
}
template <class T>
static int launch_vrows_v(lbfgsx_ctx* c, int tot, int vsel_id, int mask, const GramPrologue<T>& pro, const GramRows<T>& gr,
                          int64_t nrows, const BVecs<T>* by_pos = nullptr)
{
    if (tot <= 8) return launch_vrows<T, 8, 1>(c, tot, vsel_id, mask, pro, gr, nrows, 0, 0, by_pos);
    if (tot <= 16) return launch_vrows<T, 16, 1>(c, tot, vsel_id, mask, pro, gr, nrows, 0, 0, by_pos);
    if (tot <= 20) return launch_vrows<T, 20, 1>(c, tot, vsel_id, mask, pro, gr, nrows, 0, 0, by_pos);
    if (tot <= 24) return launch_vrows<T, 24, 1>(c, tot, vsel_id, mask, pro, gr, nrows, 0, 0, by_pos);
    return launch_vrows<T, 32, 1>(c, tot, vsel_id, mask, pro, gr, nrows, 0, 0, by_pos);
}
static int fetch_gram_out(lbfgsx_ctx* c, int first, int count, double* h)
{
    lbfgsb_state* b = c->bstate;
    if (b->gram_out_host)
    {
        LBFGSX_HIP(lbfgsx::poll_wait(c));
        const volatile double* src = b->gram_out_host + first;
        for (int i = 0; i < count; i++)
            h[i] = src[i];
        return LBFGSX_OK;
    }
    LBFGSX_HIP(lbfgsx::copy_async(h, b->gram_out + first, sizeof(double) * size_t(count), hipMemcpyDeviceToHost, c->stream));
    LBFGSX_HIP(lbfgsx::stream_sync(c->stream));
    return LBFGSX_OK;
}
static bool vrows_plan(int npairs, const int* pi, const int* pj, int tot, int NP, int& col_a, int& col_b, int* slot)
{
    int freq[kColsX + 1];
    for (int k = 0; k <= kColsX; k++)
        freq[k] = 0;
    bool other = false;
    for (int z = 0; z < npairs; z++)
        if (pi[z] != tot && pj[z] != tot)
        {
            other = true;
            freq[pi[z]]++;
            if (pj[z] != pi[z])
                freq[pj[z]]++;
        }
    col_a = col_b = -1;
    if (other)
    {
        for (int k = 0; k < tot; k++)
            if (col_a < 0 || freq[k] > freq[col_a])
                col_a = k;
        for (int k = 0; k < tot; k++)
            if (k != col_a && freq[k] > 0 && (col_b < 0 || freq[k] > freq[col_b]))
                col_b = k;
        if (col_b < 0)
            col_b = col_a;
    }
    for (int z = 0; z < npairs; z++)
    {
        const int I = pi[z], J = pj[z];
        if (I == tot || J == tot)
            slot[z] = (I == tot) ? J : I;
        else if (I == col_a || J == col_a)
            slot[z] = NP + (I == col_a ? J : I);
        else if (I == col_b || J == col_b)
            slot[z] = 2 * NP + (I == col_b ? J : I);
        else
            return false;
    }
    return true;
}
int free_delta_launch(lbfgsx_ctx* c)
{
    lbfgsb_state* b = c->bstate;
    int rc = delta_alloc(c);
    if (rc)
        return rc;
    if (!b->fd_host)
        LBFGSX_HIP(hipHostMalloc(reinterpret_cast<void**>(&b->fd_host), sizeof(unsigned) * 4, hipHostMallocDefault));
    if (b->wf_live && (!(b->wf_ncorr == c->ncorr || b->wf_ncorr + 1 == c->ncorr) || b->wf_epoch + 1 != b->sub_epoch))
        b->wf_live = false;
    const unsigned init[4] = {0u, 0u, unsigned(b->wf_live ? b->wf_n : 0), 0u};
    LBFGSX_HIP(lbfgsx::copy_async(b->dl_cnt, init, sizeof(init), hipMemcpyHostToDevice, c->stream));
    const int64_t n8 = (c->n + 7) / 8;
    const int grid = c->grid_for(n8);
    lbfgsx::model_add(double(c->n) * 2.125);
    LBFGSX_LAUNCH(k_free_delta, dim3(grid), dim3(kBlock), 0, c->stream, b->st, b->fprev, n8, c->n, b->dl_enter, b->dl_leave,
                       b->dl_cnt, b->dl_cap);
    LBFGSX_HIP(hipGetLastError());
    if (b->wf_live)
    {
        rc = upload_phys(c);
        if (rc)
            return rc;
        const int total = 2 * c->ncorr;
        int which[kColsX];
        for (int k = 0; k < total; k++)
            which[k] = k;
        DISPATCH_T(c, {
            if (total > 32)
                (void) xl::wf_append<T>(c->stream, colsx_full<T>(c, total), total, static_cast<T*>(b->wf), b->wf_ld, b->wf_idx, b->wf_pos,
                                        b->dl_enter, b->dl_cnt, b->dl_cap, unsigned(std::min<int64_t>(c->n, b->wf_ld)), c->ncorr,
                                        c->m - c->ncorr);
            else
            {
            Cols<T, 32> cl = col_list<T, 32>(c, which, total);
            LBFGSX_LAUNCH((k_wf_append<T>), dim3(16), dim3(kBlock), 0, c->stream, cl, total, static_cast<T*>(b->wf), b->wf_ld,
                               b->wf_idx, b->wf_pos, b->dl_enter, b->dl_cnt, b->dl_cap, unsigned(std::min<int64_t>(c->n, b->wf_ld)),
                               c->ncorr, c->m - c->ncorr);
            }
        });
        LBFGSX_HIP(hipGetLastError());
    }
    LBFGSX_HIP(lbfgsx::copy_async(b->fd_host, b->dl_cnt, sizeof(unsigned) * 4, hipMemcpyDeviceToHost, c->stream));
    return LBFGSX_OK;
}
static int gram_dd_core(lbfgsx_ctx* c, int mask, int vsel_id, int prologue, const double* coef1, const double* coef2,
                        double* gram, double* wtv, double* gram_dd, const int* list, int64_t nlist)
{
    int rc = need_bounded(c, false, true, true);
    if (rc)
        return rc;
    lbfgsb_state* b = c->bstate;
    b->vrow_dd_valid = false;
    const int tot = 2 * c->ncorr;
    const int ntot = tot + (vsel_id >= 0 ? 1 : 0);
    const bool lu_walk = !list && b->lu_valid && vsel_id < 0 && prologue == LBFGSX_GP_NONE && mask != 0 &&
                         (mask & ~(ST_L | ST_U)) == 0;
    {
        int slot = -1;
        if (lu_walk && mask == (ST_L | ST_U) && b->lu_n >= 1)
            slot = 0;
        else if (list && vsel_id < 0 && prologue == LBFGSX_GP_NONE && list == b->dl_enter)
            slot = 1;
        else if (list && vsel_id < 0 && prologue == LBFGSX_GP_NONE && list == b->dl_leave)
            slot = 2;
        const bool hit = slot >= 0 && !wtv && gram_stash_take(c, slot, gram, gram_dd);
        if (slot != 0)
            b->stash_valid[0] = false;
        if (hit)
            return LBFGSX_OK;
    }
    if (b->cv_live && !lu_walk)
    {
        rc = cv_back(c, false);
        if (rc)
            return rc;
    }
    if (prologue != LBFGSX_GP_NONE && (prologue < 0 || prologue > LBFGSX_GP_LINEAR))
    {
        set_error("lbfgsx_b_gram_fused_ex: the prologue needs the default one-pass Gram");
        return LBFGSX_E_INVALID;
    }
    bool wide = ntot > kGramDDCS && b->split;
    if (tot < 1 || (ntot > kGramDDCS && !wide) || b->gram_mode == 2)
    {
        set_error("lbfgsx_b_gram_fused: one-pass Gram not applicable");
        return LBFGSX_E_INVALID;
    }
    std::vector<double> hbuf(size_t(b->gtile) * 256);
    double* h = hbuf.data();
    const int npairs = ntot * (ntot + 1) / 2;
    const int kp = (npairs + 63) / 64;
    int blocks = 1;
    rc = upload_phys(c);
    if (rc)
        return rc;
    if (list)
        mask = 0;
    else if (lu_walk)
    {
        if (b->lu_n < 1)
        {
            if (gram)
                std::fill(gram, gram + size_t(tot) * size_t(tot), 0.0);
            if (gram_dd)
                std::fill(gram_dd, gram_dd + size_t(tot) * size_t(tot + 1), 0.0);
            return LBFGSX_OK;
        }
        list = b->lu_ptr();
        nlist = b->lu_n;
    }
    const bool compact_in = !list && wf_serves(c, mask);
    bool compact_out = !list && !compact_in && b->wf_use && b->wf_on && gram_dd != nullptr && mask == ST_FREE && vsel_id >= 0 &&
                       c->n < (int64_t(1) << 31) && b->nfree_last >= 4096 && b->nfree_last * 8 <= c->n * 7;
    if (compact_out)
        compact_out = wf_prepare(c);
    const int64_t nrows = list ? nlist : compact_in ? b->wf_n : c->n;
    const int64_t nbatch = (nrows + kGramDDRows - 1) / kGramDDRows;
    bool done_i8 = false;
    if (!list && b->gram_i8 && c->dtype == LBFGSX_F64 && tot <= 30 && tot >= b->i8_min_tot && (mask == 0 || (mask & ST_FREE)))
    {
        GramPrologue<double> pro;
        pro.mode = prologue;
        pro.use1 = coef1 ? 1 : 0;
        pro.use2 = coef2 ? 1 : 0;
        for (int k = 0; k < 64; k++)
// ... 213 lines not shown
    {
        rc = cv_back(c, false);
        if (rc)
            return rc;
    }
    const bool compact = wf_serves(c, mask);
    const int64_t nrows = compact ? b->wf_n : c->n;
    rc = upload_phys(c);
    if (rc)
        return rc;
    if (xsplit)
    {
        DISPATCH_T(c, {
            ProX<T> pro;
            pro.mode = prologue;
            pro.use1 = coef1 ? 1 : 0;
            pro.use2 = coef2 ? 1 : 0;
            for (int k = 0; k < kColsX; k++)
            {
                pro.c1[k] = (coef1 && k < tot) ? T(coef1[k]) : T(0);
                pro.c2[k] = (coef2 && k < tot) ? T(coef2[k]) : T(0);
            }
            RowsX<T> gr{};
            gr.in_idx = (compact && !by_pos) ? b->wf_idx : nullptr;
            const BVecs<T> cvb = bvecs_cv<T>(c);
            const ColsX<T> cl = (gr.in_idx || by_pos) ? colsx_wf<T>(c, tot) : colsx_full<T>(c, tot);
            lbfgsx::poll_arm(c);
            rc = xl::rows<T>(c->stream, b->num_cus, 1, cl, tot, by_pos ? cvb : bvecs<T>(c), vsel_id, mask, nrows, wsx(c), b->gram_out,
                             b->gram_out + 256, pro, gr, -1, -1);
        });
        if (rc)
            return rc;
        double hx[kColsX];
        rc = fetch_gram_out(c, 0, tot, hx);
        if (rc)
            return rc;
        for (int j = 0; j < tot; j++)
            wtv[j] = hx[j];
        return LBFGSX_OK;
    }
    DISPATCH_T(c, {
        GramPrologue<T> pro;
        pro.mode = prologue;
        pro.use1 = coef1 ? 1 : 0;
        pro.use2 = coef2 ? 1 : 0;
        for (int k = 0; k < 64; k++)
        {
            pro.c1[k] = (coef1 && k < tot) ? T(coef1[k]) : T(0);
            pro.c2[k] = (coef2 && k < tot) ? T(coef2[k]) : T(0);
        }
        GramRows<T> gr{};
        gr.in_idx = (compact && !by_pos) ? b->wf_idx : nullptr;
        const BVecs<T> cvb = bvecs_cv<T>(c);
        lbfgsx::poll_arm(c);
        rc = launch_vrows_v<T>(c, tot, vsel_id, mask, pro, gr, nrows, by_pos ? &cvb : nullptr);
    });
    if (rc)
        return rc;
    double h[64];
    rc = fetch_gram_out(c, 0, tot, h);
    if (rc)
        return rc;
    for (int j = 0; j < tot; j++)
        wtv[j] = h[j];
    return LBFGSX_OK;
}

int lbfgsx_b_free_delta(lbfgsx_ctx* c, int64_t* n_enter, int64_t* n_leave)
{
    lbfgsx::DeviceGuard dev_guard_(c->device);
    int rc = need_bounded(c);
    if (rc)
        return rc;
    lbfgsb_state* b = c->bstate;
    const bool ahead = b->fd_ahead && b->fd_epoch == b->sub_epoch;
    b->fd_ahead = false;
    if (!ahead)
    {
        rc = free_delta_launch(c);
        if (rc)
            return rc;
        LBFGSX_HIP(lbfgsx::stream_sync(c->stream));
    }
    const unsigned* h = b->fd_host;
    for (int d = 0; d < 2; d++)
        b->dl_n[d] = (h[d] <= b->dl_cap) ? int64_t(h[d]) : -1;
    if (b->wf_live)
    {
        if (h[3])
            b->wf_live = false;
        else
            b->wf_n = int64_t(h[2]);
    }
    *n_enter = b->dl_n[0];
    *n_leave = b->dl_n[1];
    return LBFGSX_OK;
}

int lbfgsx_b_gram_list_dd(lbfgsx_ctx* c, int which, double* gram_dd)
{
    lbfgsx::DeviceGuard dev_guard_(c->device);
    int rc = need_bounded(c, false, false, true);
    if (rc)
        return rc;
    lbfgsb_state* b = c->bstate;
    if (which < 0 || which > 1 || !b->fprev || b->dl_n[which] < 1 || !gram_dd)
    {
        set_error("lbfgsx_b_gram_list_dd: no such list (lbfgsx_b_free_delta first; an overflowed or empty list has no Gram)");
        return LBFGSX_E_INVALID;
    }
    return gram_dd_core(c, 0, -1, LBFGSX_GP_NONE, nullptr, nullptr, nullptr, nullptr, gram_dd, which == 0 ? b->dl_enter : b->dl_leave,
                        b->dl_n[which]);
}

int lbfgsx_b_gram_pairs_max(lbfgsx_ctx* c)
{
    if (!c || !c->bstate)
        return 0;
    const lbfgsb_state* b = c->bstate;
    const int tot = 2 * c->ncorr;
    if (tot < 1 || tot > kColsX || b->gram_mode == 2)
        return 0;
    if (b->split)
        return 3 * (tot + 1);
    return tot + 1 <= kGramDDCS ? 64 : 0;
}

int lbfgsx_b_gram_pairs_dd(lbfgsx_ctx* c, int mask, int vsel_id, int prologue, const double* coef1, const double* coef2,
                           int npairs, const int* pair_i, const int* pair_j, int refresh_slot, double* out_dd)
{
    lbfgsx::DeviceGuard dev_guard_(c->device);
    int rc = need_bounded(c);
    if (rc)
        return rc;
    lbfgsb_state* b = c->bstate;
    const int tot = 2 * c->ncorr, ntot = tot + 1;
    const bool xsplit = b->split;
    if (tot < 1 || tot > kColsX || vsel_id < 0 || !out_dd || b->gram_mode == 2 || npairs < 1 ||
        (xsplit ? npairs > 3 * (kColsX + 1) : (npairs > 64 || ntot > kGramDDCS)) || prologue < LBFGSX_GP_NONE || prologue > LBFGSX_GP_LINEAR)
    {
        set_error("lbfgsx_b_gram_pairs_dd: needs the default one-pass Gram, 1 <= 2c <= 80, a vector selector and 1..3 (2c + 1) entries");
        return LBFGSX_E_INVALID;
    }
    for (int e = 0; e < npairs; e++)
        if (pair_i[e] < 0 || pair_i[e] > tot || pair_j[e] < 0 || pair_j[e] > tot)
        {
            set_error("lbfgsx_b_gram_pairs_dd: entry outside the [Y S v] columns");
            return LBFGSX_E_INVALID;
        }
    if (refresh_slot < -2 || refresh_slot >= c->ncorr)
    {
        set_error("lbfgsx_b_gram_pairs_dd: refresh_slot is a storage slot, -1 (nothing replaced) or -2 (no kept copy)");
        return LBFGSX_E_INVALID;
    }
    const bool same_hist = b->wf_ncorr == c->ncorr || (b->wf_ncorr + 1 == c->ncorr && refresh_slot == c->ncorr - 1);
    const bool kept = refresh_slot >= -1 && b->wf_live && b->wf_use && mask == ST_FREE && b->wf_n * 8 <= b->nfree_last * 9 &&
                      b->wf_n >= b->nfree_last && same_hist && b->wf_epoch + 1 == b->sub_epoch;
    if (!kept)
        b->wf_live = false;
    const bool compact_in = kept || wf_serves(c, mask);
    bool compact_out = !compact_in && b->wf_use && b->wf_on && mask == ST_FREE &&
                       c->n < (int64_t(1) << 31) && b->nfree_last >= 4096 && b->nfree_last * 8 <= c->n * 7;
    rc = upload_phys(c);
    if (rc)
        return rc;
    if (compact_out)
        compact_out = wf_prepare(c);
// ... 215 lines not shown
```

lbfgspp_amd/csrc/lbfgsb_kernels.cuh:

```cuda
#pragma once
#include "reduce.cuh"

#ifndef LBFGSX_VROWS_OCC
#define LBFGSX_VROWS_OCC 2
#endif
#ifndef LBFGSX_SWEEP_OCC
#define LBFGSX_SWEEP_OCC 2
#endif
#ifndef LBFGSX_VROWS_W2
#define LBFGSX_VROWS_W2 0
#endif


namespace lbfgsx {

enum : unsigned char
{
    ST_FREE = 1,
    ST_NEWACT = 2,
    ST_L = 4,
    ST_U = 8,
    ST_P = 16
};

// ... 614 lines not shown
            acc[k].add_prod(w[k], a);
            acc[NC + k].add_prod(w[k], d);
        }
    }
    if (grid_reduce<2 * NC>(acc, ws) && threadIdx.x == 0)
    {
        for (int k = 0; k < 2 * NC; k++)
            out[k] = double(T(acc[k].value()));
        ws_signal(ws);
    }
}

template <class T, int TB>
__global__ void __launch_bounds__(kBlock) k_gram(Cols<T, TB> ci, int ni, Cols<T, TB> cj, int nj,
                                                 const unsigned char* __restrict__ st, int mask, int64_t n,
                                                 RedWs ws, double* __restrict__ out)
{
    typedef typename AccOf<T>::type A;
    A acc[TB * TB];
    const int64_t stride = int64_t(gridDim.x) * kBlock;
    for (int64_t i = int64_t(blockIdx.x) * kBlock + threadIdx.x; i < n; i += stride)
    {
        if (mask && !(st[i] & mask))
            continue;
        T vi[TB], vj[TB];
#pragma unroll
        for (int a = 0; a < TB; a++)
        {
            vi[a] = (a < ni) ? ci.p[a][i] : T(0);
            vj[a] = (a < nj) ? cj.p[a][i] : T(0);
        }
#pragma unroll
        for (int a = 0; a < TB; a++)
#pragma unroll
            for (int c = 0; c < TB; c++)
                acc[a * TB + c].add_prod(vi[a], vj[c]);
    }
    if (grid_reduce<TB * TB>(acc, ws) && threadIdx.x == 0)
        for (int k = 0; k < TB * TB; k++)
            out[k] = double(T(acc[k].value()));
}

enum { GP_NONE = 0, GP_RHS = 1, GP_LINEAR = 2 };
template <class T>
struct GramPrologue
{
    int mode;
    int use1, use2;
    T c1[64], c2[64];
};

constexpr int kGramDDRows = 64;
constexpr int kGramDDCS = 31;

constexpr int gram_dd_cs(int kp) { return kp <= 1 ? 11 : kp <= 2 ? 15 : kp <= 4 ? 23 : kp <= 6 ? 27 : 31; }
inline size_t gram_dd_lds_bytes(int cs, int kp)
{
    const size_t tile = size_t(kBlock / 64) * kGramDDRows * size_t(cs) * sizeof(double);
    const size_t scr = size_t(kBlock / 64) * size_t(kp) * 64 * 2 * sizeof(double);
    return tile > scr ? tile : scr;
}

template <class T>
struct GramRows
{
    const int* in_idx;
    T* out_w;
    int64_t out_ld;
    int out_split, out_gap;
    int* out_idx;
    const int* out_base;
    int vgroups;
    int w_by_row;
    int use_table;
    unsigned char ti[64], tj[64];
    int* out_pos;
    int fresh_a, fresh_b;
    const T *src_a, *src_b;
    T *dst_a, *dst_b;
    const unsigned char* st_alt;
    const int* st_pos;
};

template <class T>
__global__ void __launch_bounds__(kBlock) k_wf_append(Cols<T, 32> orig, int ncols, T* __restrict__ wf, int64_t wf_ld,
                                                      int* __restrict__ wf_idx, int* __restrict__ pos, const int* __restrict__ enter,
                                                      unsigned* __restrict__ cnt, unsigned cap, unsigned wf_cap, int split, int gap)
{
    const unsigned ne = __hip_atomic_load(cnt + 0, __ATOMIC_RELAXED, __HIP_MEMORY_SCOPE_AGENT);
    if (ne > cap)
    {
        if (blockIdx.x == 0 && threadIdx.x == 0)
            cnt[3] = 1u;
        return;
    }
    for (unsigned e = blockIdx.x * kBlock + threadIdx.x; e < ne; e += gridDim.x * kBlock)
    {
        const int row = enter[e];
        if (pos[row] >= 0)
            continue;
        const unsigned slot = atomicAdd(cnt + 2, 1u);
        if (slot >= wf_cap)
        {
            cnt[3] = 1u;
            continue;
        }
        wf_idx[slot] = row;
        pos[row] = int(slot);
        for (int k = 0; k < ncols; k++)
            wf[int64_t(k + (k >= split ? gap : 0)) * wf_ld + slot] = orig.p[k][row];
    }
}

static __global__ void __launch_bounds__(kBlock) k_free_delta(const unsigned char* __restrict__ st, unsigned char* __restrict__ prev,
                                                       int64_t n8 , int64_t n,
                                                       int* __restrict__ enter, int* __restrict__ leave,
                                                       unsigned* __restrict__ cnt, unsigned cap)
{
    constexpr int CAPB = 1024;
    __shared__ int s_buf[2][CAPB];
    __shared__ unsigned s_n[2], s_base[2];
    if (threadIdx.x < 2)
        s_n[threadIdx.x] = 0;
    __syncthreads();
    const int64_t stride = int64_t(gridDim.x) * kBlock;
    const int lane = threadIdx.x & 63;
    const unsigned long long* s8 = reinterpret_cast<const unsigned long long*>(st);
    unsigned long long* p8 = reinterpret_cast<unsigned long long*>(prev);
    for (int64_t v0 = (int64_t(blockIdx.x) * kBlock + threadIdx.x - lane); v0 < n8; v0 += stride)
    {
        const int64_t v = v0 + lane;
        unsigned long long now = 0, was = 0;
        if (v < n8)
        {
            now = s8[v] & 0x0101010101010101ull;
            was = p8[v];
            const int64_t left = n - v * 8;
            if (left < 8)
                now &= (1ull << (8 * left)) - 1ull;
        }
        const unsigned long long diff = now ^ was;
        if (__ballot(diff != 0ull) == 0ull)
            continue;
        if (diff)
            p8[v] = now;
#pragma unroll
        for (int dir = 0; dir < 2; dir++)
        {
            const unsigned long long bits = (dir == 0) ? (now & ~was) : (was & ~now);
            const int mine = __popcll(bits);
            int incl = mine;
#pragma unroll
            for (int off = 1; off < 64; off <<= 1)
            {
                const int o = __shfl_up(incl, off, 64);
                if (lane >= off)
                    incl += o;
            }
            const int total = __shfl(incl, 63, 64);
            if (total == 0)
                continue;
            unsigned lb = 0;
            if (lane == 63)
                lb = atomicAdd(&s_n[dir], unsigned(total));
            lb = unsigned(__shfl(int(lb), 63, 64));
            const unsigned first_over = lb > unsigned(CAPB) ? lb : unsigned(CAPB);
            const unsigned n_over = lb + unsigned(total) > first_over ? lb + unsigned(total) - first_over : 0u;
            unsigned gbase = 0;
            bool direct = false;
            if (n_over)
            {
                direct = !(__hip_atomic_load(cnt + dir, __ATOMIC_RELAXED, __HIP_MEMORY_SCOPE_AGENT) > cap);
                if (direct)
                {
                    if (lane == 63)
                        gbase = atomicAdd(cnt + dir, n_over);
                    gbase = unsigned(__shfl(int(gbase), 63, 64));
                }
            }
            unsigned pos = lb + unsigned(incl - mine);
            int* dst = (dir == 0) ? enter : leave;
#pragma unroll
            for (int k = 0; k < 8; k++)
                if ((bits >> (8 * k)) & 1ull)
                {
                    if (pos < unsigned(CAPB))
                        s_buf[dir][pos] = int(v * 8 + k);
                    else if (direct && gbase + (pos - first_over) < cap)
                        dst[gbase + (pos - first_over)] = int(v * 8 + k);
                    pos++;
                }
        }
    }
    __syncthreads();
    for (int dir = 0; dir < 2; dir++)
    {
        const unsigned held = s_n[dir], m = held < unsigned(CAPB) ? held : unsigned(CAPB);
        if (m == 0)
            continue;
        if (threadIdx.x == 0)
            s_base[dir] = atomicAdd(cnt + dir, m);
        __syncthreads();
        const unsigned base = s_base[dir];
        int* dst = (dir == 0) ? enter : leave;
        for (unsigned j = threadIdx.x; j < m; j += kBlock)
            if (base + j < cap)
                dst[base + j] = s_buf[dir][j];
    }
}

static __global__ void __launch_bounds__(kBlock) k_free_counts(const unsigned char* __restrict__ st, int64_t n, int64_t nbatch,
                                                        int* __restrict__ counts)
{
    const int lane = threadIdx.x & 63;
    const int64_t nwaves = int64_t(gridDim.x) * (kBlock / 64);
    for (int64_t bt = int64_t(blockIdx.x) * (kBlock / 64) + (threadIdx.x >> 6); bt <= nbatch; bt += nwaves)
    {
        const int64_t r = bt * 64 + lane;
        const bool keep = bt < nbatch && r < n && (st[r] & ST_FREE);
        const unsigned long long bal = __ballot(keep);
        if (lane == 0)
            counts[bt] = __popcll(bal);
    }
}

template <class T, int KP, int CS = gram_dd_cs(KP), bool VONLY = false>
__global__ void __launch_bounds__(kBlock) k_gram_dd(Cols<T, 32> cols, int ncols, BVecs<T> b, int vsel_id, int mask,
                                                    int64_t n, double* __restrict__ partial, GramPrologue<T> pro,
                                                    GramRows<T> gr)
{
    constexpr int cs = CS;
    extern __shared__ double tile[];
    __shared__ T pc1[64], pc2[64];
    if (pro.mode != GP_NONE)
    {
        if (threadIdx.x < 64)
        {
            pc1[threadIdx.x] = pro.c1[threadIdx.x];
            pc2[threadIdx.x] = pro.c2[threadIdx.x];
        }
        __syncthreads();
    }
    const int tid = threadIdx.x, lane = tid & 63, wv = tid >> 6;
    const int ntot = ncols + (vsel_id >= 0 ? 1 : 0);
    const int npairs = ntot * (ntot + 1) / 2;
    double* tl = tile + wv * (kGramDDRows * cs);
    int pi[KP], pj[KP];
    const int vg = (VONLY && gr.vgroups != 1 && !gr.use_table && 64 / ntot > 0) ? 64 / ntot : 1;
    const int grp = (VONLY && !gr.use_table) ? lane / ntot : 0;
#pragma unroll
    for (int k = 0; k < KP; k++)
    {
        int e = lane * KP + k;
        if (VONLY)
        {
            pi[k] = gr.use_table ? int(gr.ti[lane]) : ncols;
            pj[k] = gr.use_table ? int(gr.tj[lane]) : lane - grp * ntot;
            continue;
        }
        if (e >= npairs)
            e = 0;
        int I = 0;
        while ((I + 1) * (I + 2) / 2 <= e)
            I++;
        pi[k] = I;
        pj[k] = e - I * (I + 1) / 2;
    }
    DD acc0[KP], acc1[KP];
    const int64_t nbatch = (n + kGramDDRows - 1) / kGramDDRows;
    const int64_t nwaves = int64_t(gridDim.x) * (kBlock / 64);
    for (int64_t bt0 = int64_t(blockIdx.x) * (kBlock / 64) + wv; bt0 < nbatch; bt0 += 4 * nwaves)
    {
    unsigned char st4[4];
#pragma unroll
    for (int u = 0; u < 4; u++)
    {
        const int64_t ru = (bt0 + u * nwaves) * kGramDDRows + lane;
        if (mask && ru < n)
        {
            const int64_t rw = gr.in_idx ? int64_t(gr.in_idx[ru]) : ru;
            st4[u] = gr.st_alt ? gr.st_alt[gr.st_pos[rw]] : b.st[rw];
        }
        else
            st4[u] = (unsigned char) 0;
    }
#pragma unroll
    for (int u = 0; u < 4; u++)
    {
        const int64_t bt = bt0 + u * nwaves;
        if (bt >= nbatch)
            break;
// ... 621 lines not shown
        for (int k = 0; k < W; k++)
            pp[k] = pos ? pos[vi * W + k] : 0;
        Pack<T> ps, py, pt, pd, pk;
#pragma unroll
        for (int k = 0; k < W; k++)
            row(vi * W + k, px.e[k], pg_.e[k], plo.e[k], pup.e[k], pxp.e[k], pgp.e[k], pp[k], ps.e[k], py.e[k], pt.e[k], pd.e[k],
                pk.e[k]);
        stv(s, vi, ps);
        stv(y, vi, py);
        stv(b.brk, vi, pt);
        stv(b.dvec, vi, pd);
        stv(b.xcp, vi, px);
        if (keys)
            stv(keys, vi, pk);
        if (vals)
        {
#pragma unroll
            for (int k = 0; k < W; k++)
                vals[vi * W + k] = int(vi * W + k);
        }
    }
    if (blockIdx.x == 0 && threadIdx.x == 0)
        for (int64_t i = nv * W; i < n; i++)
        {
            T si, yi, t, di, key;
            row(i, b.x0[i], b.g[i], b.lb[i], b.ub[i], xp[i], gp[i], pos ? pos[i] : 0, si, yi, t, di, key);
            s[i] = si;
            y[i] = yi;
            b.brk[i] = t;
            b.dvec[i] = di;
            b.xcp[i] = b.x0[i];
            if (keys)
                keys[i] = key;
            if (vals)
                vals[i] = int(i);
        }
    if (pos)
        lu_flush_lds(s_ob, &s_on, &s_lbase, olist, ocnt, ocap);
    if (plist)
        lu_flush_lds(s_pb, &s_pn, &s_lbase, plist, pcnt, pcap);
    ext_publish<false>(pg, ws, 14);
    if (grid_reduce<7>(acc, ws))
    {
        const double pgmax = ext_collect<false>(ws, 14);
        if (threadIdx.x == 0)
        {
            const T sy = T(acc[1].value()), yy = T(acc[2].value());
            out_post[0] = T(acc[0].value());
            out_post[1] = sy;
            out_post[2] = yy;
            out_post[3] = T(pgmax);
            *ys_slot = sy;
            *theta_slot = yy / sy;
            out[0] = double(T(acc[3].value()));
            out[1] = acc[4].value();
            out[2] = acc[5].value();
            out[3] = pos ? double(__hip_atomic_load(ocnt, __ATOMIC_RELAXED, __HIP_MEMORY_SCOPE_AGENT)) : -1.0;
            if (pos)
                __hip_atomic_store(ocnt, 0u, __ATOMIC_RELAXED, __HIP_MEMORY_SCOPE_AGENT);
            out[4] = plist ? double(__hip_atomic_load(pcnt, __ATOMIC_RELAXED, __HIP_MEMORY_SCOPE_AGENT)) : -1.0;
            if (plist)
                __hip_atomic_store(pcnt, 0u, __ATOMIC_RELAXED, __HIP_MEMORY_SCOPE_AGENT);
            out[5] = acc[6].value();
            ws_signal(ws);
        }
    }
}

template <class T>
__global__ void __launch_bounds__(kBlock) k_keys_from_brk(const T* __restrict__ brk, T* __restrict__ keys, int* __restrict__ vals,
                                                         int64_t n)
{
    const T inf = T(__longlong_as_double(0x7FF0000000000000ll));
    const int64_t stride = int64_t(gridDim.x) * kBlock;
    for (int64_t i = int64_t(blockIdx.x) * kBlock + threadIdx.x; i < n; i += stride)
    {
        const T t = brk[i];
        keys[i] = (t == T(0) || t == inf) ? inf : t;
        if (vals)
            vals[i] = int(i);
    }
}

template <class T>
__global__ void k_cauchy_gather(BVecs<T> b, const T* __restrict__ keys, const int* __restrict__ vals,
                                int64_t first, int64_t count, const T* __restrict__ S, const T* __restrict__ Y,
                                int64_t ld, const int* __restrict__ phys, int ncorr, double* __restrict__ o_brk,
                                double* __restrict__ o_g, double* __restrict__ o_z, int* __restrict__ o_idx,
                                double* __restrict__ o_w)
{
    const int64_t stride = int64_t(gridDim.x) * blockDim.x;
    for (int64_t k = int64_t(blockIdx.x) * blockDim.x + threadIdx.x; k < count; k += stride)
    {
        const int idx = vals[first + k];
        o_brk[k] = double(keys[first + k]);
        o_g[k] = double(b.g[idx]);
        const T bound = (b.dvec[idx] > T(0)) ? b.ub[idx] : b.lb[idx];
        o_z[k] = double(bound - b.x0[idx]);
        o_idx[k] = idx;
        for (int j = 0; j < ncorr; j++)
        {
            o_w[k * 2 * ncorr + j] = double(Y[int64_t(phys[j]) * ld + idx]);
            o_w[k * 2 * ncorr + ncorr + j] = double(S[int64_t(phys[j]) * ld + idx]);
        }
    }
}

__device__ inline void lu_append_capped(bool app, int64_t i, int* __restrict__ lu_list, unsigned* __restrict__ lu_cnt, unsigned lu_cap)
{
    const unsigned long long am = __ballot(app);
    if (am)
    {
        const int leader = __ffsll((long long) am) - 1;
        unsigned basep = 0;
        if (int(threadIdx.x & 63) == leader)
        {
            basep = __hip_atomic_load(lu_cnt, __ATOMIC_RELAXED, __HIP_MEMORY_SCOPE_AGENT);
            if (basep <= lu_cap)
                basep = atomicAdd(lu_cnt, unsigned(__popcll(am)));
        }
        basep = unsigned(__shfl(int(basep), leader, 64));
        const unsigned pos = basep + unsigned(__popcll(am & ((1ull << (threadIdx.x & 63)) - 1ull)));
        if (app && pos < lu_cap)
            lu_list[pos] = int(i);
    }
}

template <class T>
__global__ void __launch_bounds__(kBlock) k_cauchy_finish(BVecs<T> b, T t_cross, T tfinal, int crossed_all, int64_t n,
                                                          RedWs ws, double* __restrict__ out, T* __restrict__ drt,
                                                          int* __restrict__ na_list, unsigned* __restrict__ na_cnt, unsigned na_cap)
{
    typedef typename AccOf<T>::type A;
    constexpr int W = Vec16<T>::W;
    A acc[2];
    __shared__ int s_nb[kListBuf];
    __shared__ unsigned s_nn, s_lbase;
    if (threadIdx.x == 0)
        s_nn = 0;
    __syncthreads();
    auto row = [&](int64_t i, T t, T x0i, T di, T& xc, unsigned char& s) __attribute__((always_inline)) {
        xc = x0i;
        if (t == T(0))
            s = 0;
        else if (t <= t_cross)
        {
            xc = (di > T(0)) ? b.ub[i] : b.lb[i];
            s = ST_NEWACT;
            acc[0].add(T(1));
        }
        else
        {
            if (!crossed_all)
                xc = x0i + tfinal * di;
            s = ST_FREE;
            acc[1].add(T(1));
        }
    };
    const int64_t nv = n / W;
    const int64_t stride = int64_t(gridDim.x) * kBlock;
    for (int64_t vi = int64_t(blockIdx.x) * kBlock + threadIdx.x; vi < nv; vi += stride)
    {
        const Pack<T> pt = ldv(b.brk, vi), px0 = ldv(b.x0, vi), pd = ldv(b.dvec, vi);
        Pack<T> pxc, pdr;
        unsigned char s[W];
#pragma unroll
        for (int k = 0; k < W; k++)
        {
            row(vi * W + k, pt.e[k], px0.e[k], pd.e[k], pxc.e[k], s[k]);
            pdr.e[k] = pxc.e[k] - px0.e[k];
        }
        stv(b.xcp, vi, pxc);
        if (drt)
            stv(drt, vi, pdr);
        if (W == 2)
            reinterpret_cast<unsigned short*>(b.st)[vi] = (unsigned short) (unsigned(s[0]) | (unsigned(s[1]) << 8));
        else
            reinterpret_cast<unsigned*>(b.st)[vi] = unsigned(s[0]) | (unsigned(s[1 % W]) << 8) | (unsigned(s[2 % W]) << 16) |
                                                     (unsigned(s[3 % W]) << 24);
        if (na_list)
        {
#pragma unroll
            for (int k = 0; k < W; k++)
                lu_append_lds<true>(s[k] == ST_NEWACT, vi * W + k, s_nb, &s_nn, na_list, na_cnt, na_cap);
        }
    }
    if (blockIdx.x == 0 && threadIdx.x == 0)
        for (int64_t i = nv * W; i < n; i++)
// ... 630 lines not shown
```

lbfgspp_amd/csrc/lbfgsb_state.hpp:

```cpp
#pragma once
#include <algorithm>
#include <atomic>
#include <cmath>
#include <cstdlib>
#include <cstdio>
#include <cstring>
#include <limits>
#include <vector>

#include "ctx.hpp"
#include "lbfgsb_kernels.cuh"
#include "lbfgsb_x.hpp"

struct lbfgsb_state
{
    void *brk = nullptr, *dvec = nullptr, *cF = nullptr, *y = nullptr, *yfb = nullptr, *lam = nullptr, *mu = nullptr,
         *rhs = nullptr;
    unsigned char* st = nullptr;
    void *keys_in = nullptr, *keys_out = nullptr;
    int *vals_in = nullptr, *vals_out = nullptr;
    bool keys_valid = false;
    bool vals_iota = false;
    void* sort_tmp = nullptr;
    size_t sort_tmp_bytes = 0;
// ... 12 lines not shown
    bool stash_valid[3] = {false, false, false};
    bool stash_armed[3] = {false, false, false};
    unsigned stash_phys[3] = {0, 0, 0};
    int stash_tot[3] = {0, 0, 0};
    int64_t stash_hits = 0;
    void* coef_dev = nullptr;
    int* lu_list = nullptr;
    int lu_cur = 0;
    int* lu_ptr() const { return lu_list + size_t(lu_cur) * size_t(lu_cap); }
    int* lu_other() const { return lu_list + size_t(1 - lu_cur) * size_t(lu_cap); }
    bool lu_pending = false;
    int64_t lu_pending_n = 0;
    unsigned* lu_cnt = nullptr;
    unsigned lu_cap = 0;
    int lu_n = 0;
    int64_t lu_pred = int64_t(1) << 40;
    static constexpr int64_t kLuMax = 262144;
    bool lu_valid = false;
    bool sweep_fuse = true;
    void* wf = nullptr;
    int64_t wf_ld = 0;
    int* wf_idx = nullptr;
    int* wf_cnt = nullptr;
    int* wf_base = nullptr;
    void* wf_tmp = nullptr;
    size_t wf_tmp_bytes = 0;
    bool wf_use = true;
    bool force_pending = false;
    bool pb_use = true;
    bool st_use = true;
    double vrow_dd[2 * 80];
    bool vrow_dd_valid = false;
    bool rhs_identity = true;
    bool pb_valid = false;
    int pb_cur = -1;
    double pb_tau = 0.0;
    bool pb_wc = false, pb_sel_inline = false;
    double pb_r[6] = {0, 0, 0, -1, -1, 0};
    bool psel_use = true;
    int* psel_list = nullptr;
    unsigned* psel_cnt = nullptr;
    unsigned psel_cap = 1u << 21;
    void* psel_tmp = nullptr;
    size_t psel_tmp_bytes = 0;
    int64_t psel_last = -1;
    bool list12 = true;
    bool psel_small = true;
    static constexpr int64_t kPselMax = int64_t(1) << 17;
    bool wtdc_use = true;
    int* wtdc_list = nullptr;
    unsigned* wtdc_cnt = nullptr;
    unsigned wtdc_cap = 1u << 16;
    int64_t wtdc_n = -1;
    int64_t wtdc_runs = 0;
    bool cv_use = true;
    bool cv_live = false;
    void* cv_buf = nullptr;
    int64_t cv_cap = 0;
    int64_t cv_backs = 0, cv_starts = 0;
    bool wf_on = false;
    bool wf_valid = false;
    int64_t wf_n = 0;
    int64_t nfree_last = 0;
    hipEvent_t chain_ev[8] = {nullptr, nullptr, nullptr, nullptr, nullptr, nullptr, nullptr, nullptr};
    static constexpr int kChainPieces = 8;
    unsigned char* fprev = nullptr;
    int* dl_enter = nullptr;
    int* dl_leave = nullptr;
    unsigned* dl_cnt = nullptr;
    unsigned dl_cap = 0;
    int64_t dl_n[2] = {0, 0};
    bool wf_live = false;
    int wf_ncorr = 0;
    long long sub_epoch = 0;
    long long wf_epoch = -2;
    long long wf_patched_epoch = -2;
    int wf_patched_slot = -1;
    int* wf_pos = nullptr;
    double* g_host = nullptr;
    bool gpre_use = true;
    bool fd_use = true, fd_ahead = false;
    long long fd_epoch = -1;
    unsigned* fd_host = nullptr;
    bool gpre_valid = false;
    int64_t gpre_count = 0;
    int gpre_nc = -1;
    size_t g_host_cap = 0;
    double *g_brk = nullptr, *g_g = nullptr, *g_z = nullptr, *g_w = nullptr;
    int* g_idx = nullptr;
    int64_t g_cap = 0;
    int g_ncorr = 0;
    double* gram_partial = nullptr;
    double* gram_partial2 = nullptr;
    double* gram_out = nullptr;
    static constexpr int kGramBlocks = 1024;
    bool gram_i8 = false;
    int i8_min_tot = 1;
    unsigned long long* colmax = nullptr;
    std::vector<unsigned char> colmax_ok;
    long long* i8_part = nullptr;
    double* i8_partv = nullptr;
    unsigned long long* i8_vsum = nullptr;
    int i8_waves = 0, i8_nepad = 0;
    int gram_mode = 0;
    int num_cus = 256;
    static constexpr int kDotsGrid = 512;
    bool multidot_chunked = false;
    double *s_brk = nullptr, *s_g = nullptr, *s_z = nullptr, *s_W = nullptr, *s_P = nullptr, *s_C = nullptr,
           *s_fpp = nullptr, *s_dfp = nullptr, *s_fp = nullptr, *s_ts = nullptr, *s_off = nullptr, *s_small = nullptr;
    unsigned long long* s_exit = nullptr;
    unsigned long long* exit_map_host = nullptr;
    unsigned long long* exit_map_dev = nullptr;
    double* gout_host = nullptr;
    double* gout_dev = nullptr;
    double* s_chain = nullptr;
    double* h_chain = nullptr;
    bool chain_host = true;
    int64_t s_cap = 0;
    int s_nc = 0;
    void* pk = nullptr;
    int* pv = nullptr;
    unsigned* pcount = nullptr;
    void* sel_tmp = nullptr;
    size_t sel_tmp_bytes = 0;
    bool split = true;
    double* xp1 = nullptr;
    double* xp2 = nullptr;
    unsigned* xtickets = nullptr;
    int gtile = 3;
    bool fin_fuse = true;
    bool drt_ready = false;
    int* na_list = nullptr;
    unsigned* na_cnt = nullptr;
    unsigned na_cap = 1u << 16;
    int64_t na_n = -1;
    int64_t na_prev = -1;
    static constexpr int kDout = 640;
};

#define copy_async(...) copy_async_at("copy@" LBFGSB_TU ":" LBFGSX_STR(__LINE__), __VA_ARGS__)

namespace lbfgsx {

#define DISPATCH_T(c, ...)            \
    do                                \
    {                                 \
        if ((c)->dtype == LBFGSX_F64) \
        {                             \
            typedef double T;         \
            __VA_ARGS__               \
        }                             \
        else                          \
        {                             \
            typedef float T;          \
            __VA_ARGS__               \
        }                             \
    } while (0)

template <class T>
inline T* P(void* p) { return static_cast<T*>(p); }

template <class T>
inline BVecs<T> bvecs(lbfgsx_ctx* c)
{
    lbfgsb_state* b = c->bstate;
    BVecs<T> v;
    v.x0 = P<T>(c->xb[c->cur]);
// ... 127 lines not shown
```

lbfgspp_amd/csrc/lbfgsb_x.cuh:

```cuda
#pragma once
#include "lbfgsb_kernels.cuh"
#include "reduce_x.cuh"

namespace lbfgsx {

constexpr int kColsX = 80;
static_assert(kColsX == 2 * LBFGSX_MAX_M_BOUNDED, "include/lbfgsx.h documents the cap");
constexpr int kGramSelfFinish = 16;

template <class T>
struct ColsX
{
    const T* p[kColsX];
};
template <class T>
struct ProX
{
    int mode, use1, use2;
    T c1[kColsX], c2[kColsX];
};
template <class T>
struct CoefX
{
    T c[kColsX];
// ... 1186 lines not shown
        }
    }
    if (fin_out)
    {
#pragma unroll
        for (int k = 0; k < KPB; k++)
        {
            const int e = tid * KPB + k;
            fin_out[e] = acc0[k].value();
            if (fin_dd)
            {
                fin_dd[e * 2 + 0] = acc0[k].hi;
                fin_dd[e * 2 + 1] = acc0[k].lo;
            }
        }
        if (done)
        {
            out_fence_sys();
            __syncthreads();
            if (tid == 0)
                __hip_atomic_store(done, seq, __ATOMIC_RELAXED, __HIP_MEMORY_SCOPE_SYSTEM);
        }
        return;
    }
    double* part = partial + size_t(blockIdx.x) * (KPB * 256) * 2;
#pragma unroll
    for (int k = 0; k < KPB; k++)
    {
        const int e = tid * KPB + k;
        part[e * 2 + 0] = acc0[k].hi;
        part[e * 2 + 1] = acc0[k].lo;
    }
}

static __global__ void __launch_bounds__(kBlock) kx_gram_finish(const double* __restrict__ partial, int nblocks, double* __restrict__ out,
                                                         int final, double* __restrict__ out_dd, unsigned long long* done,
                                                         unsigned long long seq, unsigned* __restrict__ ticket)
{
    const int tb = blockIdx.x, ntile = gridDim.x, ch = blockIdx.y, nch = gridDim.y, e = threadIdx.x;
    DD t;
    for (int bk = ch; bk < nblocks; bk += nch)
    {
        const double* p = partial + (size_t(bk) * ntile * 256 + size_t(tb) * 256 + e) * 2;
        t.merge(p[0], p[1]);
    }
    if (final)
    {
        out[tb * 256 + e] = t.value();
        if (out_dd)
        {
            out_dd[(tb * 256 + e) * 2 + 0] = t.hi;
            out_dd[(tb * 256 + e) * 2 + 1] = t.lo;
        }
        if (done)
        {
            out_fence_sys();
            __syncthreads();
            if (e == 0)
            {
                bool lastb = true;
                if (ntile > 1)
                {
                    const unsigned old = __hip_atomic_fetch_add(ticket, 1u, __ATOMIC_ACQ_REL, __HIP_MEMORY_SCOPE_AGENT);
                    lastb = (old == unsigned(ntile - 1));
                    if (lastb)
                        __hip_atomic_store(ticket, 0u, __ATOMIC_RELAXED, __HIP_MEMORY_SCOPE_AGENT);
                }
                if (lastb)
                    __hip_atomic_store(done, seq, __ATOMIC_RELAXED, __HIP_MEMORY_SCOPE_SYSTEM);
            }
        }
    }
    else
    {
        double* q = out + (size_t(ch) * ntile * 256 + size_t(tb) * 256 + e) * 2;
        q[0] = t.hi;
        q[1] = t.lo;
    }
}

template <class T>
__global__ void __launch_bounds__(kBlock) kx_wf_append(ColsX<T> orig, int ncols, T* __restrict__ wf, int64_t wf_ld,
                                                       int* __restrict__ wf_idx, int* __restrict__ pos, const int* __restrict__ enter,
                                                       unsigned* __restrict__ cnt, unsigned cap, unsigned wf_cap, int split, int gap)
{
    __shared__ const T* s_col[kColsX];
    if (threadIdx.x < kColsX)
        s_col[threadIdx.x] = orig.p[threadIdx.x];
    __syncthreads();
    const unsigned ne = __hip_atomic_load(cnt + 0, __ATOMIC_RELAXED, __HIP_MEMORY_SCOPE_AGENT);
    if (ne > cap)
    {
        if (blockIdx.x == 0 && threadIdx.x == 0)
            cnt[3] = 1u;
        return;
    }
    for (unsigned e = blockIdx.x * kBlock + threadIdx.x; e < ne; e += gridDim.x * kBlock)
    {
        const int row = enter[e];
        if (pos[row] >= 0)
            continue;
        const unsigned slot = atomicAdd(cnt + 2, 1u);
        if (slot >= wf_cap)
        {
            cnt[3] = 1u;
            continue;
        }
        wf_idx[slot] = row;
        pos[row] = int(slot);
        for (int k = 0; k < ncols; k++)
            wf[int64_t(k + (k >= split ? gap : 0)) * wf_ld + slot] = ((gptr_x<T>) s_col[k])[row];
    }
}

}
```

lbfgspp_amd/csrc/lbfgsb_x.hip:

```cpp
#include <algorithm>
#include <cstdlib>

#include "lbfgsb_x.hpp"

namespace lbfgsx {
namespace xl {

#ifndef LBFGSX_X40
#define LBFGSX_X40(CALL) CALL(10, 4)
#endif
#define LBFGSX_XCLASS(ncols, CALL)             \
    do                                         \
    {                                          \
        if ((ncols) <= 8) { CALL(4, 2); }      \
        else if ((ncols) <= 12) { CALL(6, 2); }  \
        else if ((ncols) <= 16) { CALL(8, 2); }  \
        else if ((ncols) <= 20) { CALL(10, 2); } \
        else if ((ncols) <= 24) { CALL(12, 2); } \
        else if ((ncols) <= 32) { CALL(8, 4); }  \
        else if ((ncols) <= 40) { LBFGSX_X40(CALL); } \
        else if ((ncols) <= 48) { CALL(12, 4); } \
        else if ((ncols) <= 60) { CALL(15, 4); } \
        else { CALL(20, 4); }                  \
    } while (0)
// ... 146 lines not shown
    constexpr int dots_per_cu = 1;
#define CALL(NCL, G)                                                                                                          \
    LBFGSX_LAUNCH((kx_multidot2_wf<T, NCL, G>),                                                                               \
                  dim3(grid_rows(std::max<int64_t>(npos, nlist), 64 / G, std::min(dots_per_cu, occ_dots_x(NCL)), num_cus)),   \
                  dim3(kBlock), 0, s, wfc, ncols, fresh_a, fresh_b, snew, ynew, dvec, idx, npos, full, list, nlist, ws, out, dst_a, dst_b)
    LBFGSX_XCLASS(ncols, CALL);
#undef CALL
    LBFGSX_HIP(hipGetLastError());
    return LBFGSX_OK;
}

template <class T>
int multidot2(hipStream_t s, int num_cus, const ColsX<T>& cols, int ncols, const T* v1, const T* v2, int64_t n, const RedWsX& ws,
              double* out)
{
    if (ncols < 1 || ncols > kColsX)
        return LBFGSX_E_INVALID;
    model_add(double(n) * (ncols + 2) * sizeof(T));
#define CALL(NCL, G)                                                                                                        \
    LBFGSX_LAUNCH((kx_multidot2<T, NCL, G>), dim3(grid_rows(n, 64 / G, occ_dots_x(NCL), num_cus)), dim3(kBlock), 0, s, cols, ncols, \
                  v1, v2, n, ws, out)
    LBFGSX_XCLASS(ncols, CALL);
#undef CALL
    LBFGSX_HIP(hipGetLastError());
    return LBFGSX_OK;
}

template <class T>
int list2(hipStream_t s, int num_cus, const ColsX<T>& cols, int ncols, const BVecs<T>& b, const int* list, int nlist, const RedWsX& ws,
          double* out, const unsigned char* stc, const int* pos, double* out_c, double* out_c_dd)
{
    if (ncols < 1 || ncols > kColsX || (out_c != nullptr) != (out_c_dd != nullptr))
        return LBFGSX_E_INVALID;
    model_add(double(nlist) * (64.0 * (ncols + 3 + (out_c ? 1 : 0)) + 4 + 64));
#define CALL(NCL, G)                                                                                                      \
    if (out_c)                                                                                                            \
        LBFGSX_LAUNCH((kx_list2<T, NCL, G, true>), dim3(std::min(32, grid_rows(nlist, 64 / G, 1, num_cus))), dim3(kBlock), 0, s, \
                      cols, ncols, b, list, nlist, ws, out, stc, pos, out_c, out_c_dd);                                   \
    else                                                                                                                  \
        LBFGSX_LAUNCH((kx_list2<T, NCL, G, false>), dim3(std::min(32, grid_rows(nlist, 64 / G, 1, num_cus))), dim3(kBlock), 0, s, \
                      cols, ncols, b, list, nlist, ws, out, stc, pos, out_c, out_c_dd)
    LBFGSX_XCLASS(ncols, CALL);
#undef CALL
    LBFGSX_HIP(hipGetLastError());
    return LBFGSX_OK;
}

template <class T>
int list1(hipStream_t s, int num_cus, const ColsX<T>& cols, int ncols, const BVecs<T>& b, int vsel_id, int mask, const int* list, int nlist,
          const RedWsX& ws, double* out, const unsigned char* stc, const int* pos, double* out_dd)
{
    if (ncols < 1 || ncols > kColsX)
        return LBFGSX_E_INVALID;
    model_add(double(nlist) * (64.0 * (ncols + 1) + 4 + 64));
#define CALL(NCL, G)                                                                                                      \
    LBFGSX_LAUNCH((kx_list1<T, NCL, G>), dim3(std::min(32, grid_rows(nlist, 64 / G, 1, num_cus))), dim3(kBlock), 0, s, cols,   \
                  ncols, b, vsel_id, mask, list, nlist, ws, out, stc, pos, out_dd)
    LBFGSX_XCLASS(ncols, CALL);
#undef CALL
    LBFGSX_HIP(hipGetLastError());
    return LBFGSX_OK;
}

template <class T>
int multidot_mask(hipStream_t s, int num_cus, const ColsX<T>& cols, int ncols, const BVecs<T>& b, int vsel_id, const T* vcol, int mask,
                  int64_t n, const RedWsX& ws, double* out)
{
    if (ncols < 1 || ncols > kColsX)
        return LBFGSX_E_INVALID;
    const int64_t want = (n + int64_t(kWaves) * 256 - 1) / (int64_t(kWaves) * 256);
    model_add(double(n));
#define CALL(NCL, G)                                                                                                   \
    LBFGSX_LAUNCH((kx_multidot_mask<T, NCL, G>),                                                                        \
                  dim3(int(std::max<int64_t>(1, std::min<int64_t>(want, std::min(occ_mask_x(NCL) * num_cus, kMaxGridX))))), \
                  dim3(kBlock), 0, s, cols, ncols, b, vsel_id, vcol, mask, n, ws, out)
    LBFGSX_XCLASS(ncols, CALL);
#undef CALL
    LBFGSX_HIP(hipGetLastError());
    return LBFGSX_OK;
}

template <class T>
int wf_append(hipStream_t s, const ColsX<T>& orig, int ncols, T* wf, int64_t wf_ld, int* wf_idx, int* pos, const int* enter,
              unsigned* cnt, unsigned cap, unsigned wf_cap, int split, int gap)
{
    LBFGSX_LAUNCH((kx_wf_append<T>), dim3(16), dim3(kBlock), 0, s, orig, ncols, wf, wf_ld, wf_idx, pos, enter, cnt, cap, wf_cap, split,
                  gap);
    LBFGSX_HIP(hipGetLastError());
    return LBFGSX_OK;
}

int gram_kpb(int ntot)
{
    const int npairs = ntot * (ntot + 1) / 2;
    const int kp = (npairs + 255) / 256;
    return kp <= 1 ? 1 : kp <= 2 ? 2 : kp <= 3 ? 3 : kp <= 4 ? 4 : kp <= 6 ? 6 : kp <= 9 ? 9 : 13;
}

template <class T, int KPB>
static int gram_kp(hipStream_t s, int max_blocks, const ColsX<T>& cols, int ncols, const BVecs<T>& b, int vsel_id, int mask,
                   int64_t n, double* partial, const ProX<T>& pro, const GramRows<T>& gr, double* fin_out, double* fin_dd,
                   unsigned long long* done, unsigned long long seq, unsigned* ticket)
{
    const int ntot = ncols + (vsel_id >= 0 ? 1 : 0);
    const int cs = ntot | 1;
    const size_t lds = size_t(64) * size_t(cs) * sizeof(double) + 64 * sizeof(int);
    if (lds > 48 * 1024)
        (void) hipFuncSetAttribute(reinterpret_cast<const void*>(kx_gram<T, KPB>), hipFuncAttributeMaxDynamicSharedMemorySize, 64 * 1024);
    const int64_t nbatch = (n + 63) / 64;
    const int blocks = int(std::max<int64_t>(1, std::min<int64_t>(max_blocks, nbatch)));
    {
        const double e = sizeof(T);
        if (gr.w_by_row && gr.in_idx)
            model_add(double(n) * (64.0 * ncols + 4 + 64));
        else
            model_add(double(n) * (double(ncols) * e * (gr.out_w ? 2 : 1) + 1 + (gr.in_idx ? 4 : 0) + (vsel_id >= 0 ? e : 0) +
                                   (gr.out_w ? 8 : 0)));
    }
    LBFGSX_LAUNCH((kx_gram<T, KPB>), dim3(blocks), dim3(kBlock), lds, s, cols, ncols, b, vsel_id, mask, n, partial, pro, gr, cs,
                  (blocks <= kGramSelfFinish && ticket) ? fin_out : static_cast<double*>(nullptr), fin_dd, done, seq, ticket);
    if (hipGetLastError() != hipSuccess)
        return -1;
    return blocks;
}

template <class T>
int gram(hipStream_t s, int max_blocks, const ColsX<T>& cols, int ncols, const BVecs<T>& b, int vsel_id, int mask, int64_t n,
         double* partial, const ProX<T>& pro, const GramRows<T>& gr, double* fin_out, double* fin_dd, unsigned long long* done,
         unsigned long long seq, unsigned* ticket)
{
    if (ncols < 1 || ncols > kColsX)
        return -1;
#define GK(K) return gram_kp<T, K>(s, max_blocks, cols, ncols, b, vsel_id, mask, n, partial, pro, gr, fin_out, fin_dd, done, seq, ticket)
    switch (gram_kpb(ncols + (vsel_id >= 0 ? 1 : 0)))
    {
    case 1: GK(1);
    case 2: GK(2);
    case 3: GK(3);
    case 4: GK(4);
    case 6: GK(6);
    case 9: GK(9);
    default: GK(13);
    }
#undef GK
}

int gram_finish(hipStream_t s, const double* partial, int blocks, int ntile, double* partial2, double* out, double* out_dd,
                unsigned long long* done, unsigned long long seq, unsigned* ticket)
{
    const int nch = std::min(blocks, 32);
    if (blocks > 1)
    {
        LBFGSX_LAUNCH(kx_gram_finish, dim3(ntile, nch), dim3(kBlock), 0, s, partial, blocks, partial2, 0, static_cast<double*>(nullptr),
                      static_cast<unsigned long long*>(nullptr), 0ull, ticket);
        LBFGSX_LAUNCH(kx_gram_finish, dim3(ntile, 1), dim3(kBlock), 0, s, partial2, nch, out, 1, out_dd, done, seq, ticket);
    }
    else
        LBFGSX_LAUNCH(kx_gram_finish, dim3(ntile, 1), dim3(kBlock), 0, s, partial, 1, out, 1, out_dd, done, seq, ticket);
    LBFGSX_HIP(hipGetLastError());
    return LBFGSX_OK;
}

#define INST(T)                                                                                                                  \
    template int rows<T>(hipStream_t, int, int, const ColsX<T>&, int, const BVecs<T>&, int, int, int64_t, const RedWsX&, double*,    \
                         double*, const ProX<T>&, const RowsX<T>&, int, int);                                                    \
    template int solve_sweep<T>(hipStream_t, int, int, const ColsX<T>&, int, const BVecs<T>&, const BVecs<T>&, int, const CoefX<T>&, \
                                int, T, int64_t, const RedWsX&, double*, int*, unsigned*, unsigned, const int*, T*, T*, int,     \
                                const ProX<T>*);                                                                                 \
    template int multidot2_wf<T>(hipStream_t, int, const ColsX<T>&, int, int, int, const T*, const T*, const T*, const int*, int64_t, \
                                 const ColsX<T>&, const int*, int, const RedWsX&, double*, T*, T*);                              \
    template int multidot2<T>(hipStream_t, int, const ColsX<T>&, int, const T*, const T*, int64_t, const RedWsX&, double*);        \
    template int list2<T>(hipStream_t, int, const ColsX<T>&, int, const BVecs<T>&, const int*, int, const RedWsX&, double*,         \
                          const unsigned char*, const int*, double*, double*);                                                   \
    template int list1<T>(hipStream_t, int, const ColsX<T>&, int, const BVecs<T>&, int, int, const int*, int, const RedWsX&,         \
                          double*, const unsigned char*, const int*, double*);                                                   \
    template int multidot_mask<T>(hipStream_t, int, const ColsX<T>&, int, const BVecs<T>&, int, const T*, int, int64_t,            \
                                  const RedWsX&, double*);                                                                       \
    template int gram<T>(hipStream_t, int, const ColsX<T>&, int, const BVecs<T>&, int, int, int64_t, double*, const ProX<T>&,      \
                         const GramRows<T>&, double*, double*, unsigned long long*, unsigned long long, unsigned*);                                                                                    \
    template int wf_append<T>(hipStream_t, const ColsX<T>&, int, T*, int64_t, int*, int*, const int*, unsigned*, unsigned, unsigned, int, \
                              int)
INST(double);
INST(float);
#undef INST

}
}
```

lbfgspp_amd/csrc/lbfgsb_x.hpp:

```cpp
#pragma once
#include "ctx.hpp"
#include "lbfgsb_x.cuh"

namespace lbfgsx {
namespace xl {

template <class T>
int rows(hipStream_t s, int num_cus, int na, const ColsX<T>& cols, int ncols, const BVecs<T>& b, int vsel_id, int mask, int64_t n,
         const RedWsX& ws, double* out, double* out_dd, const ProX<T>& pro, const RowsX<T>& gr, int col_a, int col_b);
template <class T>
int solve_sweep(hipStream_t s, int num_cus, int first, const ColsX<T>& cols, int ncols, const BVecs<T>& b, const BVecs<T>& bw,
                int vsel_id, const CoefX<T>& coef, int has_w, T theta, int64_t n, const RedWsX& ws, double* out, int* lu_list,
                unsigned* lu_cnt, unsigned lu_cap, const int* ridx, T* cli, T* cui, int cv, const ProX<T>* pro = nullptr);
template <class T>
int multidot2_wf(hipStream_t s, int num_cus, const ColsX<T>& wfc, int ncols, int fresh_a, int fresh_b, const T* snew, const T* ynew,
                 const T* dvec, const int* idx, int64_t npos, const ColsX<T>& full, const int* list, int nlist, const RedWsX& ws,
                 double* out, T* dst_a = nullptr, T* dst_b = nullptr);
template <class T>
int multidot2(hipStream_t s, int num_cus, const ColsX<T>& cols, int ncols, const T* v1, const T* v2, int64_t n, const RedWsX& ws,
              double* out);
template <class T>
int list2(hipStream_t s, int num_cus, const ColsX<T>& cols, int ncols, const BVecs<T>& b, const int* list, int nlist, const RedWsX& ws,
          double* out, const unsigned char* stc, const int* pos, double* out_c = nullptr, double* out_c_dd = nullptr);
template <class T>
int list1(hipStream_t s, int num_cus, const ColsX<T>& cols, int ncols, const BVecs<T>& b, int vsel_id, int mask, const int* list, int nlist,
          const RedWsX& ws, double* out, const unsigned char* stc = nullptr, const int* pos = nullptr, double* out_dd = nullptr);
template <class T>
int multidot_mask(hipStream_t s, int num_cus, const ColsX<T>& cols, int ncols, const BVecs<T>& b, int vsel_id, const T* vcol, int mask,
                  int64_t n, const RedWsX& ws, double* out);
template <class T>
int wf_append(hipStream_t s, const ColsX<T>& orig, int ncols, T* wf, int64_t wf_ld, int* wf_idx, int* pos, const int* enter,
              unsigned* cnt, unsigned cap, unsigned wf_cap, int split, int gap);
int gram_kpb(int ntot);
template <class T>
int gram(hipStream_t s, int max_blocks, const ColsX<T>& cols, int ncols, const BVecs<T>& b, int vsel_id, int mask, int64_t n,
         double* partial, const ProX<T>& pro, const GramRows<T>& gr, double* fin_out = nullptr, double* fin_dd = nullptr,
         unsigned long long* done = nullptr, unsigned long long seq = 0, unsigned* ticket = nullptr);
int gram_finish(hipStream_t s, const double* partial, int blocks, int ntile, double* partial2, double* out, double* out_dd,
                unsigned long long* done, unsigned long long seq, unsigned* ticket);

}
}
```

Measured before the change: 89.26 iterations/s.

## Fold delta-count and Cauchy-gather host copies into kernels via mapped memory

The free-set delta kernels now reset their counters on the device and have the last block write the four counts directly to mapped, coherent host memory. This removes a host-to-device init copy and a device-to-host readback per call. The small Cauchy gather writes its output straight into mapped pinned memory and takes the physical column map as a kernel argument, replacing the separate upload and copy. Subspace-min environment switches are read once per solver instead of on every call. The cost is extra device-side atomics and fences, and a dependence on host-coherent writes landing before the host reads.

```diff
diff --git a/include/LBFGSB.h b/include/LBFGSB.h
--- a/include/LBFGSB.h
+++ b/include/LBFGSB.h
@@ -175,7 +175,7 @@
             const auto t_sub = std::chrono::steady_clock::now();
             {
                 detail::Range range_sub("lbfgsb:subspace_min");
-                SubspaceMin<Scalar>::subspace_minimize(m_bfgs, gcp, m_param.max_submin, &st);
+                SubspaceMin<Scalar>::subspace_minimize(m_bfgs, gcp, m_param.max_submin, &st, m_sub_switches);
             }
             m_stats.submin_s += std::chrono::duration<double>(std::chrono::steady_clock::now() - t_sub).count();
             m_stats.submin_calls++;
@@ -199,6 +199,7 @@
         return !(e && e[0] == '0');
     }();
     const bool m_trace_phases = std::getenv("LBFGSX_TRACE_PHASES") != nullptr;
+    const typename SubspaceMin<Scalar>::Switches m_sub_switches = SubspaceMin<Scalar>::Switches::from_env();
 
 public:
     LBFGSBSolver(const LBFGSBParam<Scalar>& param) : m_param(param) { m_param.check_param(); }
diff --git a/include/LBFGSpp/SubspaceMin.h b/include/LBFGSpp/SubspaceMin.h
--- a/include/LBFGSpp/SubspaceMin.h
+++ b/include/LBFGSpp/SubspaceMin.h
@@ -46,7 +46,19 @@
         return true;
     }
 
+    static bool env_on(const char* name)
+    {
+        const char* e = std::getenv(name);
+        return !(e && e[0] == '0');
+    }
+
 public:
+    struct Switches
+    {
+        bool fuse;
+        bool one_sided;
+        static Switches from_env() { return Switches{env_on("LBFGSX_SUB_FUSE"), env_on("LBFGSX_LU_ONE_SIDED")}; }
+    };
     struct Stats
     {
         int sweeps = 0;
@@ -55,7 +67,7 @@
     };
 
     static void subspace_minimize(const BFGSMatB<Scalar>& bfgs, const typename Cauchy<Scalar>::Result& gcp, int maxit,
-                                  Stats* stats = nullptr)
+                                  Stats* stats = nullptr, const Switches& sw = Switches::from_env())
     {
         lbfgsx_ctx* c = bfgs.ctx();
         const Scalar theta = bfgs.theta();
@@ -67,10 +79,7 @@
         std::vector<double> lcoef;
         const bool has_lin = linear_coef(bfgs, gcp, lcoef);
         bfgs.gram_cache_reset();
-        const char* fuse_env = std::getenv("LBFGSX_SUB_FUSE");
-        const bool fuse = !(fuse_env && fuse_env[0] == '0');
-        const char* os_env = std::getenv("LBFGSX_LU_ONE_SIDED");
-        const bool one_sided = !(os_env && os_env[0] == '0');
+        const bool fuse = sw.fuse, one_sided = sw.one_sided;
         std::int64_t s7[7] = {0, 0, 0, 0, 0, 0, 0};
         bool swept = false;
         if (fuse)
diff --git a/include/lbfgsx.h b/include/lbfgsx.h
--- a/include/lbfgsx.h
+++ b/include/lbfgsx.h
@@ -148,6 +148,7 @@
 int lbfgsx_b_dg_maxstep(lbfgsx_ctx* c, double* dg, double* step_max);
 int lbfgsx_b_dg_maxstep_trial(lbfgsx_ctx* c, int objective, double step0, double* dg, double* step_max);
 int lbfgsx_b_trial_ahead_counts(const lbfgsx_ctx* c, int64_t out[2]);
+int lbfgsx_b_fold_counts(const lbfgsx_ctx* c, int64_t out[3]);
 int lbfgsx_b_post_linesearch(lbfgsx_ctx* c, double* projgnorm, double* xnorm2, double* sy, double* yy);
 int lbfgsx_b_post_linesearch_build(lbfgsx_ctx* c, double tau, double* projgnorm, double* xnorm2, double* sy, double* yy);
 int lbfgsx_b_post_build_counts(int64_t out[2], int reset);
diff --git a/lbfgspp_amd/_lib.py b/lbfgspp_amd/_lib.py
--- a/lbfgspp_amd/_lib.py
+++ b/lbfgspp_amd/_lib.py
@@ -152,6 +152,7 @@
     sig(core, "lbfgsx_b_gram_last_vrow_dd", i32, vp, pd)
     sig(core, "lbfgsx_b_wtv_lu_c", i32, vp, pd, C.POINTER(i64), pd, C.POINTER(i64), pd)
     sig(core, "lbfgsx_b_trial_ahead_counts", i32, vp, C.POINTER(i64 * 2))
+    sig(core, "lbfgsx_b_fold_counts", i32, vp, C.POINTER(i64 * 3))
     sig(core, "lbfgsx_comm_info", i32, vp, C.POINTER(i32 * 4))
     sig(core, "lbfgsx_comm_calls", i64, vp, i32)
     sig(core, "lbfgsx_comm_hook_arg", vp, vp, i32)
diff --git a/lbfgspp_amd/csrc/lbfgsb.hip b/lbfgspp_amd/csrc/lbfgsb.hip
--- a/lbfgspp_amd/csrc/lbfgsb.hip
+++ b/lbfgspp_amd/csrc/lbfgsb.hip
@@ -198,6 +198,10 @@
         b->fd_use = atoi(e) != 0;
     if (const char* e = getenv("LBFGSX_LIST12"))
         b->list12 = atoi(e) != 0;
+    if (const char* e = getenv("LBFGSX_DELTA_FOLD"))
+        b->fd_fold = atoi(e) != 0;
+    if (const char* e = getenv("LBFGSX_CHUNK_LAND"))
+        b->gland_use = atoi(e) != 0;
     if (const char* e = getenv("LBFGSX_PSEL_SMALL"))
         b->psel_small = atoi(e) != 0;
     if (const char* e = getenv("LBFGSX_SELECT_CAP"))
@@ -275,6 +279,8 @@
         (void) hipHostFree(b->g_host);
     if (b->fd_host)
         (void) hipHostFree(b->fd_host);
+    if (b->gland_host)
+        (void) hipHostFree(b->gland_host);
     (void) hipFree(b->lu_list);
     (void) hipFree(b->wf_pos);
     (void) hipFree(b->wtdc_list);
@@ -430,11 +436,14 @@
     if (!b->fprev)
     {
         b->dl_cap = unsigned(std::min<int64_t>(c->n, std::max<int64_t>(int64_t(1) << 14, std::min<int64_t>(int64_t(1) << 20, c->n / 64))));
+        if (const char* e = getenv("LBFGSX_DELTA_CAP"))
+            b->dl_cap = unsigned(std::max(1, std::min(int(b->dl_cap), atoi(e))));
         LBFGSX_HIP(hipMalloc(reinterpret_cast<void**>(&b->fprev), size_t(c->ld)));
         LBFGSX_HIP(hipMemsetAsync(b->fprev, 0, size_t(c->ld), c->stream));
         LBFGSX_HIP(hipMalloc(reinterpret_cast<void**>(&b->dl_enter), sizeof(int) * size_t(b->dl_cap)));
         LBFGSX_HIP(hipMalloc(reinterpret_cast<void**>(&b->dl_leave), sizeof(int) * size_t(b->dl_cap)));
-        LBFGSX_HIP(hipMalloc(reinterpret_cast<void**>(&b->dl_cnt), sizeof(unsigned) * 4));
+        LBFGSX_HIP(hipMalloc(reinterpret_cast<void**>(&b->dl_cnt), sizeof(unsigned) * 8));
+        LBFGSX_HIP(hipMemsetAsync(b->dl_cnt, 0, sizeof(unsigned) * 8, c->stream));
     }
     return LBFGSX_OK;
 }
@@ -475,6 +484,16 @@
     return LBFGSX_OK;
 }
 
+int lbfgsx_b_fold_counts(const lbfgsx_ctx* c, int64_t out[3])
+{
+    if (!c || !c->bstate || !out)
+        return LBFGSX_E_INVALID;
+    out[0] = c->bstate->fd_folds;
+    out[1] = c->bstate->gland_folds;
+    out[2] = c->bstate->gland_maps;
+    return LBFGSX_OK;
+}
+
 int lbfgsx_b_compact_vec_counts(int64_t out[4], int reset)
 {
     if (out)
diff --git a/lbfgspp_amd/csrc/lbfgsb_cauchy.hip b/lbfgspp_amd/csrc/lbfgsb_cauchy.hip
--- a/lbfgspp_amd/csrc/lbfgsb_cauchy.hip
+++ b/lbfgspp_amd/csrc/lbfgsb_cauchy.hip
@@ -308,21 +308,50 @@
         b->g_cap = cap;
         b->g_ncorr = c->m;
     }
-    double* d_brk = b->g_brk;
+    const size_t ndbl = size_t(count) * ((nc > 0 && with_w) ? per : size_t(3));
+    const bool land_fold = b->gland_use && c->outmap_dev && count <= lbfgsb_state::kLandCount && !idx &&
+                           c->phys.size() <= size_t(kPhysMapSlots);
+    if (land_fold && !b->gland_host)
+    {
+        LBFGSX_HIP(hipHostMalloc(reinterpret_cast<void**>(&b->gland_host), sizeof(double) * size_t(lbfgsb_state::kLandCount) * per_cap,
+                                 hipHostMallocMapped | hipHostMallocCoherent));
+        LBFGSX_HIP(hipHostGetDevicePointer(reinterpret_cast<void**>(&b->gland_dev), b->gland_host, 0));
+    }
+    double* d_brk = land_fold ? b->gland_dev : b->g_brk;
     double* d_g = d_brk + count;
     double* d_z = d_g + count;
     double* d_w = d_z + count;
+    const int grid = int(std::min<int64_t>((count + 255) / 256, 2048));
+    if (land_fold)
+    {
+        static_assert(kPhysMapSlots >= LBFGSX_MAX_M_BOUNDED + 1, "the map of a bounded context fits the kernel argument");
+        PhysMapArg pm;
+        for (size_t k = 0; k < sizeof(pm.p) / sizeof(pm.p[0]); k++)
+            pm.p[k] = k < c->phys.size() ? c->phys[k] : 0;
+        const bool stale = b->phys_seen != c->phys_version;
+        b->phys_seen = c->phys_version;
+        b->gland_folds++;
+        b->gland_maps += stale ? 1 : 0;
+        DISPATCH_T(c, {
+            BVecs<T> bv = bvecs<T>(c);
+            LBFGSX_LAUNCH((k_cauchy_gather<T, true>), dim3(grid), dim3(256), 0, c->stream, bv, P<T>(b->keys_out), b->vals_out, first,
+                               count, P<T>(c->S), P<T>(c->Y), c->ld, b->phys_dev, nc, d_brk, d_g, d_z, b->g_idx, d_w, pm,
+                               stale ? b->phys_dev : static_cast<int*>(nullptr), c->m);
+        });
+        LBFGSX_HIP(hipGetLastError());
+        *land = b->gland_host;
+        return LBFGSX_OK;
+    }
     int rc = upload_phys(c);
     if (rc)
         return rc;
-    const int grid = int(std::min<int64_t>((count + 255) / 256, 2048));
     DISPATCH_T(c, {
         BVecs<T> bv = bvecs<T>(c);
-        LBFGSX_LAUNCH((k_cauchy_gather<T>), dim3(grid), dim3(256), 0, c->stream, bv, P<T>(b->keys_out), b->vals_out, first,
-                           count, P<T>(c->S), P<T>(c->Y), c->ld, b->phys_dev, nc, d_brk, d_g, d_z, b->g_idx, d_w);
+        LBFGSX_LAUNCH((k_cauchy_gather<T, false>), dim3(grid), dim3(256), 0, c->stream, bv, P<T>(b->keys_out), b->vals_out, first,
+                           count, P<T>(c->S), P<T>(c->Y), c->ld, b->phys_dev, nc, d_brk, d_g, d_z, b->g_idx, d_w, PhysMapArg(),
+                           static_cast<int*>(nullptr), 0);
     });
     LBFGSX_HIP(hipGetLastError());
-    const size_t ndbl = size_t(count) * ((nc > 0 && with_w) ? per : size_t(3));
     if (ndbl > b->g_host_cap)
     {
         if (b->g_host)
@@ -604,6 +633,7 @@
                 const int64_t cnt = std::min<int64_t>(512, ns);
                 if (cauchy_chunk_launch(c, 0, cnt, true, nullptr, &land, nullptr) == LBFGSX_OK)
                 {
+                    b->gpre_land = land;
                     b->gpre_valid = true;
                     b->gpre_count = cnt;
                     b->gpre_nc = c->ncorr;
@@ -663,7 +693,7 @@
     const bool ahead = b->gpre_valid && first == 0 && count == b->gpre_count && nc == b->gpre_nc && !idx && (wrows || nc == 0);
     b->gpre_valid = false;
     if (ahead)
-        land = b->g_host;
+        land = b->gpre_land;
     else
     {
         rc = cauchy_chunk_launch(c, first, count, wrows != nullptr, idx, &land, &pageable);
diff --git a/lbfgspp_amd/csrc/lbfgsb_gram.hip b/lbfgspp_amd/csrc/lbfgsb_gram.hip
--- a/lbfgspp_amd/csrc/lbfgsb_gram.hip
+++ b/lbfgspp_amd/csrc/lbfgsb_gram.hip
@@ -369,17 +369,26 @@
     int rc = delta_alloc(c);
     if (rc)
         return rc;
+    const bool fold = b->fd_fold && c->outmap_dev;
     if (!b->fd_host)
-        LBFGSX_HIP(hipHostMalloc(reinterpret_cast<void**>(&b->fd_host), sizeof(unsigned) * 4, hipHostMallocDefault));
+    {
+        LBFGSX_HIP(hipHostMalloc(reinterpret_cast<void**>(&b->fd_host), sizeof(unsigned) * 4,
+                                 fold ? (hipHostMallocMapped | hipHostMallocCoherent) : hipHostMallocDefault));
+        if (fold)
+            LBFGSX_HIP(hipHostGetDevicePointer(reinterpret_cast<void**>(&b->fd_dev), b->fd_host, 0));
+    }
     if (b->wf_live && (!(b->wf_ncorr == c->ncorr || b->wf_ncorr + 1 == c->ncorr) || b->wf_epoch + 1 != b->sub_epoch))
         b->wf_live = false;
     const unsigned init[4] = {0u, 0u, unsigned(b->wf_live ? b->wf_n : 0), 0u};
-    LBFGSX_HIP(lbfgsx::copy_async(b->dl_cnt, init, sizeof(init), hipMemcpyHostToDevice, c->stream));
+    if (!fold)
+        LBFGSX_HIP(lbfgsx::copy_async(b->dl_cnt, init, sizeof(init), hipMemcpyHostToDevice, c->stream));
+    else
+        b->fd_folds++;
     const int64_t n8 = (c->n + 7) / 8;
     const int grid = c->grid_for(n8);
     lbfgsx::model_add(double(c->n) * 2.125);
     LBFGSX_LAUNCH(k_free_delta, dim3(grid), dim3(kBlock), 0, c->stream, b->st, b->fprev, n8, c->n, b->dl_enter, b->dl_leave,
-                       b->dl_cnt, b->dl_cap);
+                       b->dl_cnt, b->dl_cap, fold ? (b->wf_live ? 1 : 2) : 0, init[2], b->fd_dev);
     LBFGSX_HIP(hipGetLastError());
     if (b->wf_live)
     {
@@ -394,18 +403,19 @@
             if (total > 32)
                 (void) xl::wf_append<T>(c->stream, colsx_full<T>(c, total), total, static_cast<T*>(b->wf), b->wf_ld, b->wf_idx, b->wf_pos,
                                         b->dl_enter, b->dl_cnt, b->dl_cap, unsigned(std::min<int64_t>(c->n, b->wf_ld)), c->ncorr,
-                                        c->m - c->ncorr);
+                                        c->m - c->ncorr, fold ? b->fd_dev : static_cast<unsigned*>(nullptr));
             else
             {
             Cols<T, 32> cl = col_list<T, 32>(c, which, total);
             LBFGSX_LAUNCH((k_wf_append<T>), dim3(16), dim3(kBlock), 0, c->stream, cl, total, static_cast<T*>(b->wf), b->wf_ld,
                                b->wf_idx, b->wf_pos, b->dl_enter, b->dl_cnt, b->dl_cap, unsigned(std::min<int64_t>(c->n, b->wf_ld)),
-                               c->ncorr, c->m - c->ncorr);
+                               c->ncorr, c->m - c->ncorr, fold ? b->fd_dev : static_cast<unsigned*>(nullptr));
             }
         });
         LBFGSX_HIP(hipGetLastError());
     }
-    LBFGSX_HIP(lbfgsx::copy_async(b->fd_host, b->dl_cnt, sizeof(unsigned) * 4, hipMemcpyDeviceToHost, c->stream));
+    if (!fold)
+        LBFGSX_HIP(lbfgsx::copy_async(b->fd_host, b->dl_cnt, sizeof(unsigned) * 4, hipMemcpyDeviceToHost, c->stream));
     return LBFGSX_OK;
 }
 static int gram_dd_core(lbfgsx_ctx* c, int mask, int vsel_id, int prologue, const double* coef1, const double* coef2,
@@ -785,7 +795,7 @@
             return rc;
         LBFGSX_HIP(lbfgsx::stream_sync(c->stream));
     }
-    const unsigned* h = b->fd_host;
+    const volatile unsigned* h = b->fd_host;
     for (int d = 0; d < 2; d++)
         b->dl_n[d] = (h[d] <= b->dl_cap) ? int64_t(h[d]) : -1;
     if (b->wf_live)
diff --git a/lbfgspp_amd/csrc/lbfgsb_kernels.cuh b/lbfgspp_amd/csrc/lbfgsb_kernels.cuh
--- a/lbfgspp_amd/csrc/lbfgsb_kernels.cuh
+++ b/lbfgspp_amd/csrc/lbfgsb_kernels.cuh
@@ -720,46 +720,86 @@
     const int* st_pos;
 };
 
+__device__ __forceinline__ void delta_ticket_reset(unsigned* __restrict__ cnt)
+{
+    __hip_atomic_store(cnt + 4, 0u, __ATOMIC_RELAXED, __HIP_MEMORY_SCOPE_AGENT);
+}
+__device__ __forceinline__ void delta_flag(unsigned* __restrict__ cnt)
+{
+    __hip_atomic_store(cnt + 3, 1u, __ATOMIC_RELAXED, __HIP_MEMORY_SCOPE_AGENT);
+    __threadfence();
+}
+__device__ inline void delta_close(unsigned* __restrict__ cnt, unsigned* __restrict__ host4)
+{
+    __syncthreads();
+    if (threadIdx.x != 0)
+        return;
+    __threadfence();
+    const unsigned old = __hip_atomic_fetch_add(cnt + 4, 1u, __ATOMIC_RELAXED, __HIP_MEMORY_SCOPE_AGENT);
+    if (old != gridDim.x - 1)
+        return;
+    __threadfence();
+    delta_ticket_reset(cnt);
+    if (!host4)
+        return;
+#pragma unroll
+    for (int k = 0; k < 4; k++)
+    {
+        const unsigned v = __hip_atomic_load(cnt + k, __ATOMIC_RELAXED, __HIP_MEMORY_SCOPE_AGENT);
+        __hip_atomic_store(host4 + k, v, __ATOMIC_RELAXED, __HIP_MEMORY_SCOPE_SYSTEM);
+        if (k != 2)
+            __hip_atomic_store(cnt + k, 0u, __ATOMIC_RELAXED, __HIP_MEMORY_SCOPE_AGENT);
+    }
+    out_fence_sys();
+}
+
 template <class T>
 __global__ void __launch_bounds__(kBlock) k_wf_append(Cols<T, 32> orig, int ncols, T* __restrict__ wf, int64_t wf_ld,
                                                       int* __restrict__ wf_idx, int* __restrict__ pos, const int* __restrict__ enter,
-                                                      unsigned* __restrict__ cnt, unsigned cap, unsigned wf_cap, int split, int gap)
+                                                      unsigned* __restrict__ cnt, unsigned cap, unsigned wf_cap, int split, int gap,
+                                                      unsigned* __restrict__ host4)
 {
     const unsigned ne = __hip_atomic_load(cnt + 0, __ATOMIC_RELAXED, __HIP_MEMORY_SCOPE_AGENT);
     if (ne > cap)
     {
         if (blockIdx.x == 0 && threadIdx.x == 0)
-            cnt[3] = 1u;
-        return;
-    }
-    for (unsigned e = blockIdx.x * kBlock + threadIdx.x; e < ne; e += gridDim.x * kBlock)
-    {
-        const int row = enter[e];
-        if (pos[row] >= 0)
-            continue;
-        const unsigned slot = atomicAdd(cnt + 2, 1u);
-        if (slot >= wf_cap)
-        {
-            cnt[3] = 1u;
-            continue;
-        }
-        wf_idx[slot] = row;
-        pos[row] = int(slot);
-        for (int k = 0; k < ncols; k++)
-            wf[int64_t(k + (k >= split ? gap : 0)) * wf_ld + slot] = orig.p[k][row];
-    }
+            delta_flag(cnt);
+    }
+    else
+        for (unsigned e = blockIdx.x * kBlock + threadIdx.x; e < ne; e += gridDim.x * kBlock)
+        {
+            const int row = enter[e];
+            if (pos[row] >= 0)
+                continue;
+            const unsigned slot = atomicAdd(cnt + 2, 1u);
+            if (slot >= wf_cap)
+            {
+                delta_flag(cnt);
+                continue;
+            }
+            wf_idx[slot] = row;
+            pos[row] = int(slot);
+            for (int k = 0; k < ncols; k++)
+                wf[int64_t(k + (k >= split ? gap : 0)) * wf_ld + slot] = orig.p[k][row];
+        }
+    if (host4)
+        delta_close(cnt, host4);
 }
 
 static __global__ void __launch_bounds__(kBlock) k_free_delta(const unsigned char* __restrict__ st, unsigned char* __restrict__ prev,
                                                        int64_t n8 , int64_t n,
                                                        int* __restrict__ enter, int* __restrict__ leave,
-                                                       unsigned* __restrict__ cnt, unsigned cap)
+                                                       unsigned* __restrict__ cnt, unsigned cap,
+                                                       int fold ,
+                                                       unsigned wf_n, unsigned* __restrict__ host4)
 {
     constexpr int CAPB = 1024;
     __shared__ int s_buf[2][CAPB];
     __shared__ unsigned s_n[2], s_base[2];
     if (threadIdx.x < 2)
         s_n[threadIdx.x] = 0;
+    if (fold && blockIdx.x == 0 && threadIdx.x == 0)
+        __hip_atomic_store(cnt + 2, wf_n, __ATOMIC_RELAXED, __HIP_MEMORY_SCOPE_AGENT);
     __syncthreads();
     const int64_t stride = int64_t(gridDim.x) * kBlock;
     const int lane = threadIdx.x & 63;
@@ -845,6 +885,8 @@
             if (base + j < cap)
                 dst[base + j] = s_buf[dir][j];
     }
+    if (fold == 2)
+        delta_close(cnt, host4);
 }
 
 static __global__ void __launch_bounds__(kBlock) k_free_counts(const unsigned char* __restrict__ st, int64_t n, int64_t nbatch,
@@ -1632,13 +1674,20 @@
     }
 }
 
-template <class T>
+constexpr int kPhysMapSlots = 41;
+struct PhysMapArg
+{
+    int p[kPhysMapSlots];
+};
+template <class T, bool LAND = false>
 __global__ void k_cauchy_gather(BVecs<T> b, const T* __restrict__ keys, const int* __restrict__ vals,
                                 int64_t first, int64_t count, const T* __restrict__ S, const T* __restrict__ Y,
                                 int64_t ld, const int* __restrict__ phys, int ncorr, double* __restrict__ o_brk,
                                 double* __restrict__ o_g, double* __restrict__ o_z, int* __restrict__ o_idx,
-                                double* __restrict__ o_w)
-{
+                                double* __restrict__ o_w, PhysMapArg pmap, int* __restrict__ phys_out, int nphys)
+{
+    if (LAND && phys_out && blockIdx.x == 0 && int(threadIdx.x) < nphys)
+        phys_out[threadIdx.x] = pmap.p[threadIdx.x];
     const int64_t stride = int64_t(gridDim.x) * blockDim.x;
     for (int64_t k = int64_t(blockIdx.x) * blockDim.x + threadIdx.x; k < count; k += stride)
     {
@@ -1650,10 +1699,13 @@
         o_idx[k] = idx;
         for (int j = 0; j < ncorr; j++)
         {
-            o_w[k * 2 * ncorr + j] = double(Y[int64_t(phys[j]) * ld + idx]);
-            o_w[k * 2 * ncorr + ncorr + j] = double(S[int64_t(phys[j]) * ld + idx]);
-        }
-    }
+            const int64_t col = LAND ? int64_t(pmap.p[j]) : int64_t(phys[j]);
+            o_w[k * 2 * ncorr + j] = double(Y[col * ld + idx]);
+            o_w[k * 2 * ncorr + ncorr + j] = double(S[col * ld + idx]);
+        }
+    }
+    if (LAND)
+        out_fence_sys();
 }
 
 __device__ inline void lu_append_capped(bool app, int64_t i, int* __restrict__ lu_list, unsigned* __restrict__ lu_cnt, unsigned lu_cap)
diff --git a/lbfgspp_amd/csrc/lbfgsb_state.hpp b/lbfgspp_amd/csrc/lbfgsb_state.hpp
--- a/lbfgspp_amd/csrc/lbfgsb_state.hpp
+++ b/lbfgspp_amd/csrc/lbfgsb_state.hpp
@@ -118,7 +118,16 @@
     bool fd_use = true, fd_ahead = false;
     long long fd_epoch = -1;
     unsigned* fd_host = nullptr;
+    bool fd_fold = true;
+    unsigned* fd_dev = nullptr;
+    int64_t fd_folds = 0;
     bool gpre_valid = false;
+    double* gpre_land = nullptr;
+    bool gland_use = true;
+    static constexpr int64_t kLandCount = 512;
+    double* gland_host = nullptr;
+    double* gland_dev = nullptr;
+    int64_t gland_folds = 0, gland_maps = 0;
     int64_t gpre_count = 0;
     int gpre_nc = -1;
     size_t g_host_cap = 0;
diff --git a/lbfgspp_amd/csrc/lbfgsb_x.cuh b/lbfgspp_amd/csrc/lbfgsb_x.cuh
--- a/lbfgspp_amd/csrc/lbfgsb_x.cuh
+++ b/lbfgspp_amd/csrc/lbfgsb_x.cuh
@@ -1292,7 +1292,8 @@
 template <class T>
 __global__ void __launch_bounds__(kBlock) kx_wf_append(ColsX<T> orig, int ncols, T* __restrict__ wf, int64_t wf_ld,
                                                        int* __restrict__ wf_idx, int* __restrict__ pos, const int* __restrict__ enter,
-                                                       unsigned* __restrict__ cnt, unsigned cap, unsigned wf_cap, int split, int gap)
+                                                       unsigned* __restrict__ cnt, unsigned cap, unsigned wf_cap, int split, int gap,
+                                                       unsigned* __restrict__ host4)
 {
     __shared__ const T* s_col[kColsX];
     if (threadIdx.x < kColsX)
@@ -1302,25 +1303,27 @@
     if (ne > cap)
     {
         if (blockIdx.x == 0 && threadIdx.x == 0)
-            cnt[3] = 1u;
-        return;
-    }
-    for (unsigned e = blockIdx.x * kBlock + threadIdx.x; e < ne; e += gridDim.x * kBlock)
-    {
-        const int row = enter[e];
-        if (pos[row] >= 0)
-            continue;
-        const unsigned slot = atomicAdd(cnt + 2, 1u);
-        if (slot >= wf_cap)
-        {
-            cnt[3] = 1u;
-            continue;
-        }
-        wf_idx[slot] = row;
-        pos[row] = int(slot);
-        for (int k = 0; k < ncols; k++)
-            wf[int64_t(k + (k >= split ? gap : 0)) * wf_ld + slot] = ((gptr_x<T>) s_col[k])[row];
-    }
-}
-
-}
+            delta_flag(cnt);
+    }
+    else
+        for (unsigned e = blockIdx.x * kBlock + threadIdx.x; e < ne; e += gridDim.x * kBlock)
+        {
+            const int row = enter[e];
+            if (pos[row] >= 0)
+                continue;
+            const unsigned slot = atomicAdd(cnt + 2, 1u);
+            if (slot >= wf_cap)
+            {
+                delta_flag(cnt);
+                continue;
+            }
+            wf_idx[slot] = row;
+            pos[row] = int(slot);
+            for (int k = 0; k < ncols; k++)
+                wf[int64_t(k + (k >= split ? gap : 0)) * wf_ld + slot] = ((gptr_x<T>) s_col[k])[row];
+        }
+    if (host4)
+        delta_close(cnt, host4);
+}
+
+}
diff --git a/lbfgspp_amd/csrc/lbfgsb_x.hip b/lbfgspp_amd/csrc/lbfgsb_x.hip
--- a/lbfgspp_amd/csrc/lbfgsb_x.hip
+++ b/lbfgspp_amd/csrc/lbfgsb_x.hip
@@ -252,10 +252,10 @@
 
 template <class T>
 int wf_append(hipStream_t s, const ColsX<T>& orig, int ncols, T* wf, int64_t wf_ld, int* wf_idx, int* pos, const int* enter,
-              unsigned* cnt, unsigned cap, unsigned wf_cap, int split, int gap)
+              unsigned* cnt, unsigned cap, unsigned wf_cap, int split, int gap, unsigned* host4)
 {
     LBFGSX_LAUNCH((kx_wf_append<T>), dim3(16), dim3(kBlock), 0, s, orig, ncols, wf, wf_ld, wf_idx, pos, enter, cnt, cap, wf_cap, split,
-                  gap);
+                  gap, host4);
     LBFGSX_HIP(hipGetLastError());
     return LBFGSX_OK;
 }
@@ -349,7 +349,7 @@
     template int gram<T>(hipStream_t, int, const ColsX<T>&, int, const BVecs<T>&, int, int, int64_t, double*, const ProX<T>&,      \
                          const GramRows<T>&, double*, double*, unsigned long long*, unsigned long long, unsigned*);                                                                                    \
     template int wf_append<T>(hipStream_t, const ColsX<T>&, int, T*, int64_t, int*, int*, const int*, unsigned*, unsigned, unsigned, int, \
-                              int)
+                              int, unsigned*)
 INST(double);
 INST(float);
 #undef INST
diff --git a/lbfgspp_amd/csrc/lbfgsb_x.hpp b/lbfgspp_amd/csrc/lbfgsb_x.hpp
--- a/lbfgspp_amd/csrc/lbfgsb_x.hpp
+++ b/lbfgspp_amd/csrc/lbfgsb_x.hpp
@@ -30,7 +30,7 @@
                   int64_t n, const RedWsX& ws, double* out);
 template <class T>
 int wf_append(hipStream_t s, const ColsX<T>& orig, int ncols, T* wf, int64_t wf_ld, int* wf_idx, int* pos, const int* enter,
-              unsigned* cnt, unsigned cap, unsigned wf_cap, int split, int gap);
+              unsigned* cnt, unsigned cap, unsigned wf_cap, int split, int gap, unsigned* host4 = nullptr);
 int gram_kpb(int ntot);
 template <class T>
 int gram(hipStream_t s, int max_blocks, const ColsX<T>& cols, int ncols, const BVecs<T>& b, int vsel_id, int mask, int64_t n,
```

Result: no change. 89.20 iterations/s (-0.1%).
